# shadygm/Lichtfeld-Densification-Plugin

Measured on AMD Instinct MI355X. Metric: triangulated points/sec + pairs/sec, MipNeRF360 garden @fast, 1/2/4/8 GPU, higher is better.
Workload: dtype f32 (+f64 Sampson/DLT solve)

## Files before the change

### lichtfeld-densification-plugin_amd/csrc/lfd_api.hip

```cpp
#include <cstddef>
#include <hip/hip_runtime.h>
#include <hip/hip_ext.h>

#include <algorithm>
#include <cmath>
#include <cstdio>
#include <cstdlib>
#include <cstring>
#include <mutex>
#include <string>
#include <vector>

#include "lfd_context.hpp"
#include "lfd_corr.hpp"
#include "lfd_block.hpp"
#include "lfd_head.hpp"
#include "lfd_cycle.hpp"
#include "lfd_support.hpp"
#include "lfd_refine.hpp"
#include "lfd_normals.hpp"
#include "lfd_sigma.hpp"
#include "lfd_consensus.hpp"
#include "lfd_undistort.hpp"
#include "lfd_freespace.hpp"
#include "lfd_fuse.hpp"
#include "lfd_knn.hpp"
#include "lfd_cap.hpp"

extern "C" __global__ void lfd_aggregate_kernel(LfdLaunch L, float* best_cert, uint8_t* best_slot);
extern "C" __global__ void lfd_dense_kernel(LfdLaunch L);
extern "C" __global__ void lfd_dense_exact_kernel(LfdLaunch L);
extern "C" __global__ void lfd_dense_ply_kernel(LfdLaunch L);
extern "C" __global__ void lfd_dense_ply_exact_kernel(LfdLaunch L);
extern "C" __global__ void lfd_dense_segments_kernel(LfdLaunch L);
extern "C" __global__ void lfd_dense_segments_exact_kernel(LfdLaunch L);
extern "C" __global__ void lfd_dense_ply_segments_kernel(LfdLaunch L);
extern "C" __global__ void lfd_dense_ply_segments_exact_kernel(LfdLaunch L);
extern "C" __global__ void lfd_segment_scan_kernel(const LfdTileSeg* table, int n_tiles, int tiles_per_ref, int n_refs, long long* tile_dst, long long* ref_offsets);
extern "C" __global__ void lfd_order_segments_kernel(const long long* tile_dst, const LfdTileSeg* table, long long hw, int tiles_per_ref, int n_tiles,
                                                     const float* sxyz, const float* srgb, const float* serr, const int* scell, const unsigned char* sslot,
                                                     float* dxyz, float* drgb, float* derr, int* dcell, unsigned char* dslot, long long capacity);
extern "C" __global__ void lfd_pack_ply_segments_kernel(const long long* tile_dst, const LfdTileSeg* table, long long hw, int tiles_per_ref, int n_tiles,
                                                        const float* xyz, const float* rgb, long long capacity, unsigned char* out);
extern "C" __global__ void lfd_pack_points3d_segments_kernel(const long long* tile_dst, const LfdTileSeg* table, long long hw, int tiles_per_ref, int n_tiles,
                                                             const float* xyz, const float* rgb, const float* err, long long capacity,
                                                             unsigned long long id_base, unsigned char* out);
extern "C" __global__ void lfd_pair_setup_kernel(LfdLaunch L, LfdRefConst* ref_out, LfdPairConst* pair_out);
extern "C" __global__ void lfd_select_filter_kernel(LfdSelectArgs A);
extern "C" __global__ void lfd_pack_ply_kernel(const float* xyz, const float* rgb, long long n, unsigned char* out);
extern "C" __global__ void lfd_pack_points3d_kernel(const float* xyz, const float* rgb, const float* err, long long n,
                                                    unsigned long long id_base, unsigned char* out);
extern "C" __global__ void lfd_copy_segments_kernel(LfdCopyArgs A, const unsigned char* src, unsigned char* dst);
extern "C" __global__ void lfd_quantise_rgb_kernel(const float* rgb, long long n3, unsigned char* out);
extern "C" __global__ void lfd_voxel_minmax_kernel(const float* xyz, const float* rgb, long long n, LfdVoxStats* part);
extern "C" __global__ void lfd_voxel_final_kernel(const LfdVoxStats* part, int n_part, LfdVoxStats* out);
extern "C" __global__ void lfd_voxel_keys_kernel(const float* xyz, long long n, double o0, double o1, double o2, double vs, unsigned long long e1,
                                                 unsigned long long e2, unsigned long long* keys, unsigned* idx);
extern "C" __global__ void lfd_voxel_hist_kernel(const unsigned long long* keys, long long n, long long chunk, int shift, unsigned* counts);
extern "C" __global__ void lfd_voxel_scan_kernel(unsigned* v, int m, unsigned* total);
extern "C" __global__ void lfd_voxel_scatter_kernel(const unsigned long long* kin, const unsigned* iin, long long n, long long chunk, int shift,
                                                    const unsigned* counts, unsigned long long* kout, unsigned* iout);
extern "C" __global__ void lfd_voxel_head_count_kernel(const unsigned long long* keys, long long n, long long chunk, unsigned* counts);
extern "C" __global__ void lfd_voxel_head_scatter_kernel(const unsigned long long* keys, long long n, long long chunk, const unsigned* counts,
                                                         unsigned* vstart);
extern "C" __global__ void lfd_voxel_sums_kernel(const float* xyz, const float* rgb, long long n, const unsigned* sorted_idx, const unsigned* vstart,
                                                 const unsigned* nv_p, double cscale, float* xyz_out, float* rgb_out, unsigned* big, unsigned* n_big);
extern "C" __global__ void lfd_voxel_sums_big_kernel(const float* xyz, const float* rgb, long long n, const unsigned* sorted_idx, const unsigned* vstart,
                                                     const unsigned* nv_p, double cscale, const unsigned* big, const unsigned* n_big, float* xyz_out,
                                                     float* rgb_out);
hipError_t lfd_undistort_launch(const LfdUndistortArgs& p, unsigned long long* n_invalid, hipStream_t stream);
extern "C" __global__ void lfd_consensus_minmax_kernel(const float* xyz, long long n, LfdVoxStats* part);
extern "C" __global__ void lfd_consensus_keys_kernel(const float* xyz, long long n, double o0, double o1, double o2, double h, unsigned long long e1,
                                                     unsigned long long e2, unsigned long long sentinel, unsigned long long* keys, unsigned* idx);
extern "C" __global__ void lfd_consensus_gather_kernel(const float* xyz, const unsigned* sorted_idx, const long long* offs, int n_refs, long long n,
                                                       LfdConsensusPt* spt);
extern "C" __global__ void lfd_consensus_count_kernel(const unsigned long long* skey, const LfdConsensusPt* spt, const unsigned* sorted_idx, long long n,
                                                      unsigned long long e1, unsigned long long e2, unsigned long long sentinel, float r2, int min_refs,
                                                      int bound, uint8_t* keep, uint8_t* consensus);
extern "C" __global__ void lfd_consensus_wgcount_kernel(const uint8_t* keep, long long n, unsigned* wg_kept);
extern "C" __global__ void lfd_consensus_offsets_kernel(const long long* offs, int n_refs, const uint8_t* keep, const unsigned* wg_kept, long long* offs_out);
extern "C" __global__ void lfd_consensus_scatter_kernel(const float* xyz, const float* rgb, const float* err, long long n, const uint8_t* keep,
                                                        const unsigned* wg_kept, float* o_xyz, float* o_rgb, float* o_err);
extern "C" __global__ void lfd_fuse_side_kernel(const float* normals, long long n, const unsigned* sorted_idx, const unsigned* vstart, const unsigned* nv_p,
                                                uint8_t* flag, unsigned* rows, unsigned* big, unsigned* n_big);
extern "C" __global__ void lfd_fuse_side_big_kernel(const float* normals, long long n, const unsigned* sorted_idx, const unsigned* vstart, const unsigned* nv_p,
                                                    const unsigned* big, const unsigned* n_big, uint8_t* flag, unsigned* rows);
extern "C" __global__ void lfd_fuse_rowsum_kernel(const unsigned* rows, const unsigned* nv_p, long long chunk, unsigned* counts);
extern "C" __global__ void lfd_fuse_rowstart_kernel(unsigned* rows, const unsigned* nv_p, long long chunk, const unsigned* counts);
extern "C" __global__ void lfd_fuse_sums_kernel(const float* xyz, const float* normals, const float* rgb, long long n, const unsigned* sorted_idx,
                                                const unsigned* vstart, const unsigned* nv_p, const uint8_t* flag, const unsigned* rowstart, double cscale,
                                                float* xyz_out, float* normals_out, float* rgb_out, unsigned* count_out);
extern "C" __global__ void lfd_fuse_sums_big_kernel(const float* xyz, const float* normals, const float* rgb, long long n, const unsigned* sorted_idx,
                                                    const unsigned* vstart, const unsigned* nv_p, const uint8_t* flag, const unsigned* rowstart, double cscale,
                                                    const unsigned* big, const unsigned* n_big, float* xyz_out, float* normals_out, float* rgb_out,
                                                    unsigned* count_out);
extern "C" __global__ void lfd_knn_keys_kernel(const float* xyz, long long n, LfdKnnGrid g, unsigned long long* keys, unsigned* idx);
extern "C" __global__ void lfd_knn_cellmax_kernel(const unsigned* vstart, const unsigned* nv_p, long long n, unsigned* max_out);
extern "C" __global__ void lfd_knn_gather_kernel(const float* xyz, const unsigned* sorted_idx, long long n, LfdKnnPt* spt);
extern "C" __global__ void lfd_knn_scan_kernel(const unsigned long long* skey, const LfdKnnPt* spt, long long n, LfdKnnGrid g, float* dist2, unsigned* list,
                                               unsigned* n_list);
extern "C" __global__ void lfd_knn_brute_kernel(const LfdKnnPt* spt, long long n, const unsigned* list, const unsigned* n_list, float* dist2);
extern "C" __global__ void lfd_pack_gaussians_kernel(const float* xyz, const float* normals, const float* rgb, const float* dist2, long long n, float opacity,
                                                     double log_flatten, float max_m, float* out);
extern "C" __global__ void lfd_cap_keys_kernel(const float* xyz, long long n, LfdCapBox box, unsigned long long* keys, unsigned* idx);
extern "C" __global__ void lfd_cap_levels_kernel(const unsigned long long* keys, long long n, unsigned* hist);
extern "C" __global__ void lfd_cap_coarsen_kernel(unsigned long long* keys, long long n, int shift);
extern "C" __global__ void lfd_cap_rep_kernel(const unsigned* sorted_idx, const unsigned* vstart, const unsigned* nc_p, const float* err, long long n,
                                              unsigned long long budget, unsigned long long* rep);
extern "C" __global__ void lfd_cap_mark_kernel(const unsigned long long* rep, const unsigned* nc_p, long long n, unsigned long long budget, uint8_t* keep);
extern "C" __global__ void lfd_cap_index_kernel(const uint8_t* keep, const unsigned* wg_kept, long long n, long long capacity, long long* keep_out);
extern "C" __global__ void lfd_freespace_fill_kernel(uint32_t* zbuf, long long n_words);
extern "C" __global__ void lfd_freespace_splat_kernel(const float* xyz, long long n, const long long* offs, int n_refs, const LfdFreespaceCam* cams, int pw,
                                                      int ph, uint32_t* zbuf);
extern "C" __global__ void lfd_freespace_count_kernel(const float* xyz, long long n, const long long* offs, int n_refs, const LfdFreespaceCam* cams,
                                                      const uint32_t* zbuf, int pw, int ph, float tol, int min_violations, uint8_t* keep,
                                                      uint8_t* violations, uint8_t* supports);
hipError_t lfd_corr_launch(const LfdCorrArgs& p, hipStream_t stream);
hipError_t lfd_block_launch(const LfdBlockArgs& p, hipStream_t stream);
hipError_t lfd_head_launch(const LfdHeadArgs& p, hipStream_t stream);
hipError_t lfd_cycle_launch(const LfdCycleArgs& p, hipStream_t stream);
hipError_t lfd_support_launch(const LfdSupportArgs& p, hipStream_t stream);
hipError_t lfd_refine_launch(const LfdRefineArgs& p, hipStream_t stream);
hipError_t lfd_sigma_launch(const LfdSigmaArgs& p, hipStream_t stream);
hipError_t lfd_normals_launch(const LfdNormalArgs& p, hipStream_t stream);
extern "C" __global__ void lfd_pack_ply_normals_kernel(const float* xyz, const float* normals, const float* rgb, long long n, unsigned char* out);
extern "C" __global__ void lfd_select_topm_kernel(LfdSelectArgs A);
extern "C" __global__ void lfd_select_filter_mw_kernel(LfdSelectArgs A, LfdSelectNorms norms);
extern "C" __global__ void lfd_select_begins_kernel(long long* pairs, long long stride, int n);
extern "C" __global__ void lfd_mt_seed_kernel(unsigned* mt, unsigned seed);
extern "C" __global__ void lfd_mt_seed_batch_kernel(unsigned* mt_base, LfdSeedBatch seeds);
extern "C" __global__ void lfd_indexed_eval_kernel(LfdLaunch L, const long long* sel_idx, const long long* sel_offsets, float* scratch,
                                                   uint8_t* codes, unsigned* tab, int off_pairs);
extern "C" __global__ void lfd_indexed_kernel(LfdLaunch L, const long long* sel_idx, const long long* sel_offsets,
                                              float* scratch, uint8_t* codes, int32_t* seg_order, const unsigned* tab, int off_pairs);

namespace {

std::mutex g_create_mutex;
std::string g_create_error;
thread_local std::string t_create_error_copy;

}

namespace {

int fail(lfd_context* ctx, int code, const std::string& msg) { return lfd_fail(ctx, code, msg); }

#define LFD_HIP(ctx, expr)                                                                         \
    do {                                                                                           \
        hipError_t e_ = (expr);                                                                    \
        if (e_ != hipSuccess)                                                                      \
            return fail((ctx), LFD_ERR_HIP, std::string(#expr) + ": " + hipGetErrorString(e_));    \
    } while (0)

int ensure(lfd_context* ctx, DeviceBuffer& b, size_t bytes, bool zero = false) {
    if (b.bytes >= bytes && b.ptr) return LFD_OK;
    if (b.ptr) {
        LFD_HIP(ctx, hipStreamSynchronize(ctx->stream));
        if (ctx->prep_stream) LFD_HIP(ctx, hipStreamSynchronize(ctx->prep_stream));
        LFD_HIP(ctx, hipFree(b.ptr));
        b.ptr = nullptr; b.bytes = 0;
    }
    size_t want = std::max<size_t>(bytes, 256);
    want = (want + 255) & ~size_t(255);
    LFD_HIP(ctx, hipMalloc(&b.ptr, want));
    b.bytes = want;
    if (zero) LFD_HIP(ctx, hipMemsetAsync(b.ptr, 0, want, ctx->stream));
    return LFD_OK;
}

int validate_batch(lfd_context* ctx, const lfd_batch* b, const lfd_params* p) {
    if (!ctx) return fail(nullptr, LFD_ERR_INVALID, "null context");
    if (ctx->is_host) return fail(ctx, LFD_ERR_STATE, "this context was made by lfd_create_host: it serves the *_host entry points only");
    if (!b || !p) return fail(ctx, LFD_ERR_INVALID, "null batch/params");
    if (ctx->n_cams <= 0) return fail(ctx, LFD_ERR_STATE, "lfd_upload_cameras must be called first");
    if (b->n_refs <= 0) return fail(ctx, LFD_ERR_INVALID, "n_refs must be > 0");
    if (b->k <= 0 || b->k > LFD_MAX_SLOTS) return fail(ctx, LFD_ERR_INVALID, "k must be in [1, LFD_MAX_SLOTS]");
    if (b->H <= 0 || b->W <= 0 || b->w_match <= 1 || b->h_match <= 1) return fail(ctx, LFD_ERR_INVALID, "bad grid / match size");
    if (b->w_match >= (1 << 24) || b->h_match >= (1 << 24) || (long long)b->w_match * b->h_match * 3 > 0x7fffffffLL)
        return fail(ctx, LFD_ERR_INVALID, "match-size image too large");
    if ((long long)b->H * b->W > 0x7fffffffLL) return fail(ctx, LFD_ERR_INVALID, "grid too large");
    if (b->warp_channels != 2 && b->warp_channels != 4) return fail(ctx, LFD_ERR_INVALID, "warp_channels must be 2 or 4");
    if (!b->ref_cam || !b->n_slots || !b->nbr_cam || !b->cert || !b->warp || !b->image)
        return fail(ctx, LFD_ERR_INVALID, "null table in batch");
    if ((b->axis_x == nullptr) != (b->axis_y == nullptr)) return fail(ctx, LFD_ERR_INVALID, "axis_x and axis_y must both be given or both be null");
    for (int r = 0; r < b->n_refs; ++r) {
        if (b->ref_cam[r] < 0 || b->ref_cam[r] >= ctx->n_cams) return fail(ctx, LFD_ERR_INVALID, "ref_cam out of range");
        if (b->n_slots[r] < 1 || b->n_slots[r] > b->k) return fail(ctx, LFD_ERR_INVALID, "n_slots must be in [1, k]");
        if (!b->image[r]) return fail(ctx, LFD_ERR_INVALID, "null image pointer");
        for (int j = 0; j < b->n_slots[r]; ++j) {
            const size_t s = (size_t)r * b->k + j;
            if (b->nbr_cam[s] < 0 || b->nbr_cam[s] >= ctx->n_cams) return fail(ctx, LFD_ERR_INVALID, "nbr_cam out of range");
            if (!b->cert[s] || !b->warp[s]) return fail(ctx, LFD_ERR_INVALID, "null cert/warp pointer in a valid slot");
            if ((reinterpret_cast<uintptr_t>(b->cert[s]) & 15u) || (reinterpret_cast<uintptr_t>(b->warp[s]) & 15u))
                return fail(ctx, LFD_ERR_INVALID, "cert/warp planes must be 16-byte aligned");
        }
    }
    return LFD_OK;
}

int slot_events(lfd_context* ctx, LfdBatchSlot& sl) {
    if (!sl.pinned_free) LFD_HIP(ctx, hipEventCreateWithFlags(&sl.pinned_free, hipEventDisableTiming));
    if (!sl.ready) LFD_HIP(ctx, hipEventCreateWithFlags(&sl.ready, hipEventDisableTiming));
    if (!sl.idle) LFD_HIP(ctx, hipEventCreateWithFlags(&sl.idle, hipEventDisableTiming));
    return LFD_OK;
}

int upload_tables(lfd_context* ctx, const lfd_batch* b, const long long* extra, size_t n_extra, bool ahead, int* slot_out, hipStream_t* stream_out,
                  const LfdRefDesc** d_refs, const LfdSlotDesc** d_slots, const long long** d_extra, const float** d_fund) {
    const size_t nr = (size_t)b->n_refs, ns = nr * (size_t)b->k;
    const size_t off_slots = (nr * sizeof(LfdRefDesc) + 15) & ~size_t(15);
    const size_t off_fund = (off_slots + ns * sizeof(LfdSlotDesc) + 15) & ~size_t(15);
    const size_t total = (off_fund + (b->fundamental ? ns * 9 * sizeof(float) : 0) + 15) & ~size_t(15);
    const size_t off_extra = total;
    const size_t extra_room = ((nr + 1) * sizeof(long long) + 15) & ~size_t(15);
    std::vector<unsigned char> blob(total, 0);
    LfdRefDesc* refs = reinterpret_cast<LfdRefDesc*>(blob.data());
    LfdSlotDesc* slots = reinterpret_cast<LfdSlotDesc*>(blob.data() + off_slots);
    for (size_t r = 0; r < nr; ++r) {
        refs[r].image = b->image[r];
        refs[r].mask_a = b->mask_a ? b->mask_a[r] : nullptr;
        refs[r].cam = b->ref_cam[r];
        refs[r].n_slots = b->n_slots[r];
        refs[r].any_mask = refs[r].mask_a ? 1 : 0;
        refs[r].pad = 0;
        for (int j = 0; j < b->k; ++j) {
            LfdSlotDesc& s = slots[r * b->k + j];
            const bool valid = j < b->n_slots[r];
            s.cert = valid ? b->cert[r * b->k + j] : nullptr;
            s.warp = valid ? b->warp[r * b->k + j] : nullptr;
            s.mask_b = (valid && b->mask_b) ? b->mask_b[r * b->k + j] : nullptr;
            s.cam = valid ? b->nbr_cam[r * b->k + j] : 0;
            s.pad = 0;
            if (s.mask_b) refs[r].any_mask = 1;
        }
    }
    if (b->fundamental) std::memcpy(blob.data() + off_fund, b->fundamental, ns * 9 * sizeof(float));
    if (n_extra * sizeof(long long) > extra_room) return fail(ctx, LFD_ERR_INVALID, "internal: selection offsets beyond the reserved room");

    int si = -1;
    for (int c = 0; c < 2; ++c) {
        const int i = c == 0 ? ctx->cur : 1 - ctx->cur;
        if (ctx->slot[i].desc.ptr && ctx->slot[i].cache == blob) { si = i; break; }
    }
    hipStream_t st = ctx->stream;
    if (si >= 0) {
        LfdBatchSlot& sl = ctx->slot[si];
        if (!ahead && sl.ready_pending) {
#if !defined(LFD_EXPERIMENT_NO_READY_WAIT)
            LFD_HIP(ctx, hipStreamWaitEvent(ctx->stream, sl.ready, 0));
#endif
            sl.ready_pending = false;
        }
        if (ahead && sl.ready_pending) st = ctx->prep_stream;
    } else {
        if (ahead) {
            if (!ctx->prep_stream) LFD_HIP(ctx, hipStreamCreateWithFlags(&ctx->prep_stream, hipStreamNonBlocking));
            si = ctx->last_used < 0 ? ctx->cur : 1 - ctx->cur;
            st = ctx->prep_stream;
        } else {
            si = ctx->cur;
        }
        LfdBatchSlot& sl = ctx->slot[si];
        int rc = slot_events(ctx, sl);
        if (rc != LFD_OK) return rc;
        if (ahead) {
            if (sl.used) LFD_HIP(ctx, hipStreamWaitEvent(st, sl.idle_attached ? sl.idle_ext : sl.idle, 0));
        } else if (sl.ready_pending) {
            LFD_HIP(ctx, hipStreamWaitEvent(ctx->stream, sl.ready, 0));
            sl.ready_pending = false;
        }
        rc = ensure(ctx, sl.desc, total + extra_room);
        if (rc != LFD_OK) return rc;
        if (sl.pinned_bytes < total + extra_room) {
            if (sl.pinned_in_flight) { LFD_HIP(ctx, hipEventSynchronize(sl.pinned_free)); sl.pinned_in_flight = false; }
            if (sl.pinned) LFD_HIP(ctx, hipHostFree(sl.pinned));
            sl.pinned = nullptr;
            sl.pinned_bytes = std::max<size_t>((total + extra_room) * 2, 1 << 16);
            LFD_HIP(ctx, hipHostMalloc(&sl.pinned, sl.pinned_bytes, hipHostMallocDefault));
        }
        if (sl.pinned_in_flight) { LFD_HIP(ctx, hipEventSynchronize(sl.pinned_free)); sl.pinned_in_flight = false; }
        std::memcpy(sl.pinned, blob.data(), total);
        LFD_HIP(ctx, hipMemcpyAsync(sl.desc.ptr, sl.pinned, total, hipMemcpyHostToDevice, st));
        LFD_HIP(ctx, hipEventRecord(sl.pinned_free, st));
        sl.pinned_in_flight = true;
        sl.cache.swap(blob);
        sl.consts_valid = false;
    }
    LfdBatchSlot& sl = ctx->slot[si];
    if (n_extra) {
        if (sl.desc.bytes < total + extra_room) return fail(ctx, LFD_ERR_STATE, "internal: batch slot without room for the selection offsets");
        if (sl.x_in_flight) { LFD_HIP(ctx, hipEventSynchronize(sl.x_free)); sl.x_in_flight = false; }
        if (sl.pinned_x_bytes < extra_room) {
            if (sl.pinned_x) LFD_HIP(ctx, hipHostFree(sl.pinned_x));
            sl.pinned_x = nullptr;
            sl.pinned_x_bytes = std::max<size_t>(extra_room * 2, 4096);
            LFD_HIP(ctx, hipHostMalloc(&sl.pinned_x, sl.pinned_x_bytes, hipHostMallocDefault));
        }
        if (!sl.x_free) LFD_HIP(ctx, hipEventCreateWithFlags(&sl.x_free, hipEventDisableTiming));
        std::memcpy(sl.pinned_x, extra, n_extra * sizeof(long long));
        LFD_HIP(ctx, hipMemcpyAsync(static_cast<unsigned char*>(sl.desc.ptr) + off_extra, sl.pinned_x, n_extra * sizeof(long long), hipMemcpyHostToDevice,
                                    ctx->stream));
        LFD_HIP(ctx, hipEventRecord(sl.x_free, ctx->stream));
        sl.x_in_flight = true;
    }
    *slot_out = si;
    *stream_out = st;
    *d_refs = reinterpret_cast<const LfdRefDesc*>(sl.desc.ptr);
    *d_slots = reinterpret_cast<const LfdSlotDesc*>(static_cast<unsigned char*>(sl.desc.ptr) + off_slots);
    if (d_extra) *d_extra = reinterpret_cast<const long long*>(static_cast<unsigned char*>(sl.desc.ptr) + off_extra);
    *d_fund = b->fundamental ? reinterpret_cast<const float*>(static_cast<unsigned char*>(sl.desc.ptr) + off_fund) : nullptr;
    return LFD_OK;
}

int default_axes(lfd_context* ctx, int W, int H, const float** ax, const float** ay) {
    if (ctx->axes_w != W || ctx->axes_h != H || !ctx->axes.ptr) {
        int rc = ensure(ctx, ctx->axes, sizeof(float) * (size_t)(W + H));
        if (rc != LFD_OK) return rc;
        std::vector<float> host((size_t)W + H);
        lfd_identity_axis(W, host.data());
        lfd_identity_axis(H, host.data() + W);
        LFD_HIP(ctx, hipMemcpyAsync(ctx->axes.ptr, host.data(), host.size() * sizeof(float), hipMemcpyHostToDevice, ctx->stream));
        LFD_HIP(ctx, hipStreamSynchronize(ctx->stream));
        ctx->axes_w = W; ctx->axes_h = H;
    }
    *ax = static_cast<const float*>(ctx->axes.ptr);
    *ay = *ax + W;
    return LFD_OK;
}

int colour_tables(lfd_context* ctx, int W, int H, int wm, int hm, const LfdColourCol** cols, const LfdColourRow** rows) {
    const int key[4] = {W, H, wm, hm};
    if (!ctx->colour_tab.ptr || std::memcmp(key, ctx->colour_key, sizeof(key)) != 0) {
        static_assert(sizeof(LfdColourCol) == 16 && sizeof(LfdColourRow) == 16, "colour table entries are 16 bytes");
        int rc = ensure(ctx, ctx->colour_tab, sizeof(LfdColourCol) * (size_t)W + sizeof(LfdColourRow) * (size_t)H);
        if (rc != LFD_OK) return rc;
        std::vector<unsigned char> host(sizeof(LfdColourCol) * (size_t)W + sizeof(LfdColourRow) * (size_t)H);
        LfdColourCol* hc = reinterpret_cast<LfdColourCol*>(host.data());
        LfdColourRow* hr = reinterpret_cast<LfdColourRow*>(host.data() + sizeof(LfdColourCol) * (size_t)W);
        const LfdAxis ax = lfd_make_axis(W), ay = lfd_make_axis(H);
        for (int x = 0; x < W; ++x) hc[x] = lfd_colour_col(lfd_match_px(lfd_axis_value(ax, x), (float)(wm - 1)), wm);
        for (int y = 0; y < H; ++y) hr[y] = lfd_colour_row(lfd_match_px(lfd_axis_value(ay, y), (float)(hm - 1)), wm, hm);
        LFD_HIP(ctx, hipMemcpyAsync(ctx->colour_tab.ptr, host.data(), host.size(), hipMemcpyHostToDevice, ctx->stream));
        LFD_HIP(ctx, hipStreamSynchronize(ctx->stream));
        std::memcpy(ctx->colour_key, key, sizeof(key));
    }
    *cols = static_cast<const LfdColourCol*>(ctx->colour_tab.ptr);
    *rows = reinterpret_cast<const LfdColourRow*>(static_cast<const unsigned char*>(ctx->colour_tab.ptr) + sizeof(LfdColourCol) * (size_t)W);
    return LFD_OK;
}

}

void lfd_fill_kernel_params(const lfd_batch* b, const lfd_params* p, LfdKernelParams& kp) {
    kp.sampson_thresh = p->sampson_thresh;
    kp.certainty_thresh = p->certainty_thresh;
    kp.reproj_thresh = p->reproj_thresh;
    kp.no_filter = p->no_filter ? 1 : 0;
    (void)LFD_FLAG_EXACT_COLOUR;
    kp.use_sampson = (!p->no_filter && p->sampson_thresh > 0.0) ? 1 : 0;
    kp.use_parallax = (!p->no_filter && p->min_parallax_deg > 0.0f) ? 1 : 0;
    kp.dot_thresh = kp.use_parallax ? lfd_parallax_dot_threshold(p->min_parallax_deg) : 2.0f;
    kp.wm1 = (float)(b->w_match - 1);
    kp.hm1 = (float)(b->h_match - 1);
}

namespace {

int prepare_launch(lfd_context* ctx, const lfd_batch* b, const lfd_params* p, const long long* extra, size_t n_extra,
                   LfdLaunch& L, const long long** d_extra, bool ahead = false) {
    int rc = validate_batch(ctx, b, p);
    if (rc != LFD_OK) return rc;
    LFD_HIP(ctx, hipSetDevice(ctx->device));
    std::memset(&L, 0, sizeof(L));
    if (!ahead && ctx->last_used >= 0) {
        LfdBatchSlot& prev = ctx->slot[ctx->last_used];
        rc = slot_events(ctx, prev);
        if (rc != LFD_OK) return rc;
        if (!prev.idle_attached) LFD_HIP(ctx, hipEventRecord(prev.idle, ctx->stream));
        prev.used = true;
    }
    int si = 0;
    hipStream_t st = ctx->stream;
    rc = upload_tables(ctx, b, extra, n_extra, ahead, &si, &st, &L.refs, &L.slots, d_extra, &L.fund_override);
    if (rc != LFD_OK) return rc;
    LfdBatchSlot& sl = ctx->slot[si];
    L.cams = static_cast<const LfdCam*>(ctx->cams.ptr);
    if (b->axis_x) { L.axis_x = b->axis_x; L.axis_y = b->axis_y; }
    else {
        rc = default_axes(ctx, b->W, b->H, &L.axis_x, &L.axis_y);
        if (rc != LFD_OK) return rc;
        L.axis_identity = 1;
    }
    L.ax = lfd_make_axis(b->W);
    L.ay = lfd_make_axis(b->H);
    L.n_refs = b->n_refs; L.k = b->k; L.H = b->H; L.W = b->W;
    L.w_match = b->w_match; L.h_match = b->h_match; L.warp_channels = b->warp_channels;
    const long long HW = (long long)b->H * b->W;
    const int tile = LFD_DENSE_BLOCK * LFD_DENSE_CPT;
    L.tiles_per_ref = (int)((HW + tile - 1) / tile);
    L.mask_sx = (float)b->w_match / (float)b->W;
    L.mask_sy = (float)b->h_match / (float)b->H;
    L.inv_w = 1.0f / (float)b->W;
    L.w_log2 = -1;
    if ((b->W & (b->W - 1)) == 0) { int l = 0; while ((1 << l) < b->W) ++l; L.w_log2 = l; }
    lfd_fill_kernel_params(b, p, L.kp);
    const size_t ref_bytes = ((size_t)b->n_refs * sizeof(LfdRefConst) + 15) & ~size_t(15);
    const size_t need = ref_bytes + (size_t)b->n_refs * b->k * sizeof(LfdPairConst);
    if (sl.consts.bytes < need) sl.consts_valid = false;
    rc = ensure(ctx, sl.consts, need);
    if (rc != LFD_OK) return rc;
    LfdRefConst* d_rc = static_cast<LfdRefConst*>(sl.consts.ptr);
    LfdPairConst* d_pc = reinterpret_cast<LfdPairConst*>(static_cast<unsigned char*>(sl.consts.ptr) + ref_bytes);
    L.ref_const = d_rc;
    L.pair_const = d_pc;
    if (!sl.consts_valid || sl.wm != b->w_match || sl.hm != b->h_match) {
        const int n = b->n_refs * b->k + b->n_refs;
        hipLaunchKernelGGL(lfd_pair_setup_kernel, dim3((unsigned)((n + 63) / 64)), dim3(64), 0, st, L, d_rc, d_pc);
        LFD_HIP(ctx, hipGetLastError());
        sl.consts_valid = true;
        sl.refs = b->n_refs; sl.k = b->k;
        sl.wm = b->w_match;
        sl.hm = b->h_match;
        if (st != ctx->stream) {
            LFD_HIP(ctx, hipEventRecord(sl.ready, st));
            sl.ready_pending = true;
        }
    }
    if (!ahead) {
        ctx->cur = si; ctx->last_used = si;
        sl.idle_attached = false;
    }
    return LFD_OK;
}

constexpr size_t kWsHeader = 128 + 128 * LFD_TICKET_LANES;

int prepare_lookback(lfd_context* ctx, size_t n_tiles, size_t n_tickets, bool lanes, LfdLaunch& L) {
    const size_t need = kWsHeader + n_tiles * sizeof(unsigned long long);
    const bool fresh = ctx->ws.bytes < need || !ctx->ws.ptr;
    int rc = ensure(ctx, ctx->ws, need, true);
    if (rc != LFD_OK) return rc;
    if (fresh) {
        ctx->tickets_issued = 0; ctx->epoch = 0;
        for (int s = 0; s < LFD_TICKET_LANES; ++s) ctx->lane_issued[s] = 0;
    }
    ctx->epoch = (ctx->epoch + 1) & LFD_EPOCH_MASK;
    if (ctx->epoch == 0) {
        LFD_HIP(ctx, hipMemsetAsync(static_cast<unsigned char*>(ctx->ws.ptr) + kWsHeader, 0, ctx->ws.bytes - kWsHeader, ctx->stream));
        LFD_HIP(ctx, hipMemsetAsync(static_cast<unsigned char*>(ctx->ws.ptr) + 16, 0, 4, ctx->stream));
        ctx->epoch = 1;
    }
    unsigned char* base = static_cast<unsigned char*>(ctx->ws.ptr);
    L.ticket = reinterpret_cast<unsigned long long*>(base);
    L.ticket_lanes = reinterpret_cast<unsigned long long*>(base + 128);
    L.tile_state = reinterpret_cast<unsigned long long*>(base + kWsHeader);
    L.status = reinterpret_cast<unsigned int*>(base + 8);
    L.seg_ready = reinterpret_cast<unsigned int*>(base + 16);
    L.ticket_base = ctx->tickets_issued;
    L.epoch = ctx->epoch;
    if (lanes) {
        for (int s = 0; s < LFD_TICKET_LANES; ++s) {
            L.ticket_base_lane[s] = ctx->lane_issued[s];
            if ((size_t)s < n_tickets) ctx->lane_issued[s] += (n_tickets - (size_t)s + LFD_TICKET_LANES - 1) / LFD_TICKET_LANES;
        }
    } else {
        ctx->tickets_issued += n_tickets;
    }
    return LFD_OK;
}

void read_env_switches(lfd_context* ctx) {
    ctx->env = LfdEnvSwitches();
    if (const char* e = std::getenv("LFD_DENSE_EXTRA_LDS")) ctx->env.dense_extra_lds = (size_t)std::atol(e);
    if (const char* e = std::getenv("LFD_DENSE_TIMING")) ctx->env.dense_timing_path = e;
    if (const char* e = std::getenv("LFD_INDEXED_SPLIT")) ctx->env.indexed_split = std::atoi(e) != 0;
    if (const char* e = std::getenv("LFD_SELECT_TIMING")) ctx->env.select_timing = std::max(1, std::atoi(e));
    if (const char* e = std::getenv("LFD_SELECT_WORKGROUPS")) ctx->env.select_workgroups = std::atoi(e);
}

int check_points(lfd_context* ctx, const lfd_points* out, const long long* ref_offsets) {
    if (!out || !out->xyz || !out->rgb || !out->err) return fail(ctx, LFD_ERR_INVALID, "null output buffers");
    if (out->capacity < 0) return fail(ctx, LFD_ERR_INVALID, "negative capacity");
    if (!ref_offsets) return fail(ctx, LFD_ERR_INVALID, "ref_offsets is required");
    return LFD_OK;
}

int batch_launch(lfd_context* ctx, const lfd_batch* batch, LfdLaunch& L) {
    lfd_params none;
    std::memset(&none, 0, sizeof(none));
    return prepare_launch(ctx, batch, &none, nullptr, 0, L, nullptr);
}

struct CloudPlan {
    long long n;
    long long G, chunk;
    int n_part;
    long long n_wg;
    unsigned grid;
};

CloudPlan cloud_plan(int64_t n) {
    CloudPlan p;
    p.n = n;
    p.G = std::min<long long>(1024, (n + 4095) / 4096);
    p.chunk = (((n + p.G - 1) / p.G) + 511) / 512 * 512;
    p.G = (n + p.chunk - 1) / p.chunk;
    p.n_part = (int)std::min<long long>(1024, (n + 255) / 256);
    p.n_wg = (n + 255) / 256;
    p.grid = (unsigned)std::min<long long>(p.n_wg, 4096);
    return p;
}

struct Bump {
    unsigned char* base;
    size_t at = 0;
    template <class T>
    T* take(size_t count, size_t extra_bytes = 0) {
        const size_t o = at;
        at = (at + count * sizeof(T) + extra_bytes + 255) & ~size_t(255);
        return base ? reinterpret_cast<T*>(base + o) : nullptr;
    }
};

template <class Layout>
int carve_cloud_ws(lfd_context* ctx, Layout&& layout) {
    Bump size{nullptr};
    layout(size);
    if (int rc = ensure(ctx, ctx->cloud_ws, size.at)) return rc;
    Bump b{static_cast<unsigned char*>(ctx->cloud_ws.ptr)};
    layout(b);
    return LFD_OK;
}

struct CloudSort {
    LfdVoxStats *part, *stats;
    unsigned* counters;
    unsigned* counts;
    unsigned long long* keys[2];
    unsigned* idx[2];
    unsigned* vstart;
};

CloudSort carve_sort(Bump& b, long long n, int n_counters, bool heads) {
    CloudSort w;
    w.part = b.take<LfdVoxStats>(1024);
    w.stats = b.take<LfdVoxStats>(1, (size_t)n_counters * sizeof(unsigned));
    w.counters = w.stats ? reinterpret_cast<unsigned*>(w.stats + 1) : nullptr;
    w.counts = b.take<unsigned>(256 * 1024);
    for (int i = 0; i < 2; ++i) w.keys[i] = b.take<unsigned long long>((size_t)n);
    for (int i = 0; i < 2; ++i) w.idx[i] = b.take<unsigned>((size_t)n);
    w.vstart = heads ? b.take<unsigned>((size_t)n) : nullptr;
    return w;
}

int cloud_stats(lfd_context* ctx, const CloudPlan& p, const CloudSort& w, const float* xyz, const float* rgb, LfdVoxStats& s) {
    hipStream_t st = ctx->stream;
    if (rgb) hipLaunchKernelGGL(lfd_voxel_minmax_kernel, dim3(p.n_part), dim3(256), 0, st, xyz, rgb, p.n, w.part);
    else hipLaunchKernelGGL(lfd_consensus_minmax_kernel, dim3(p.n_part), dim3(256), 0, st, xyz, p.n, w.part);
    hipLaunchKernelGGL(lfd_voxel_final_kernel, dim3(1), dim3(256), 0, st, w.part, p.n_part, w.stats);
    LFD_HIP(ctx, hipGetLastError());
    LFD_HIP(ctx, hipMemcpyAsync(ctx->pinned_words, w.stats, sizeof(LfdVoxStats), hipMemcpyDeviceToHost, st));
    LFD_HIP(ctx, hipStreamSynchronize(st));
    std::memcpy(&s, ctx->pinned_words, sizeof(s));
    return LFD_OK;
}

int cloud_sort(hipStream_t st, const CloudPlan& p, const CloudSort& w, int bits) {
    int cur = 0;
    for (int shift = 0; shift < bits; shift += 8, cur ^= 1) {
        hipLaunchKernelGGL(lfd_voxel_hist_kernel, dim3((unsigned)p.G), dim3(256), 0, st, w.keys[cur], p.n, p.chunk, shift, w.counts);
        hipLaunchKernelGGL(lfd_voxel_scan_kernel, dim3(1), dim3(1024), 0, st, w.counts, (int)(256 * p.G), (unsigned*)nullptr);
        hipLaunchKernelGGL(lfd_voxel_scatter_kernel, dim3((unsigned)p.G), dim3(512), 0, st, w.keys[cur], w.idx[cur], p.n, p.chunk, shift, w.counts,
                           w.keys[cur ^ 1], w.idx[cur ^ 1]);
    }
    return cur;
}

void cloud_heads_count(hipStream_t st, const CloudPlan& p, const CloudSort& w, int cur) {
// ... 339 lines not shown
        if (FILE* f = std::fopen(stamp_path, "wb")) { std::fwrite(host.data(), sizeof(unsigned long long), host.size(), f); std::fclose(f); }
    }
#endif
    return LFD_OK;
}

int lfd_triangulate_dense(lfd_context* ctx, const lfd_batch* batch, const lfd_params* params, const lfd_points* out,
                          int64_t* ref_offsets, int32_t* seg_counts) {
    return dense_launch(ctx, batch, params, out, ref_offsets, seg_counts, nullptr, nullptr);
}

int lfd_triangulate_dense_ply(lfd_context* ctx, const lfd_batch* batch, const lfd_params* params, uint8_t* records, int64_t capacity,
                              int64_t* ref_offsets, int32_t* seg_counts, int32_t* cell, uint8_t* slot) {
    if (ctx && !records) return fail(ctx, LFD_ERR_INVALID, "lfd_triangulate_dense_ply: records is null");
    lfd_points out;
    std::memset(&out, 0, sizeof(out));
    out.capacity = capacity;
    out.cell = cell;
    out.slot = slot;
    return dense_launch(ctx, batch, params, &out, ref_offsets, seg_counts, nullptr, nullptr, records);
}

int lfd_dense_tiles_per_ref(int32_t H, int32_t W) {
    if (H <= 0 || W <= 0) return 0;
    const long long tile = LFD_DENSE_BLOCK * LFD_DENSE_CPT;
    return (int)(((long long)H * W + tile - 1) / tile);
}

int lfd_triangulate_dense_segments(lfd_context* ctx, const lfd_batch* batch, const lfd_params* params, const lfd_points* out,
                                   int64_t* ref_counts, int32_t* seg_counts, lfd_tile_segment* table) {
    if (ctx && !table) return fail(ctx, LFD_ERR_INVALID, "lfd_triangulate_dense_segments: the tile table is required");
    return dense_launch(ctx, batch, params, out, nullptr, seg_counts, ref_counts, table);
}

int lfd_triangulate_dense_ply_segments(lfd_context* ctx, const lfd_batch* batch, const lfd_params* params, uint8_t* records, int64_t capacity,
                                       int64_t* ref_counts, int32_t* seg_counts, lfd_tile_segment* table) {
    if (ctx && (!records || !table)) return fail(ctx, LFD_ERR_INVALID, "lfd_triangulate_dense_ply_segments: records and the tile table are required");
    lfd_points out;
    std::memset(&out, 0, sizeof(out));
    out.capacity = capacity;
    return dense_launch(ctx, batch, params, &out, nullptr, seg_counts, ref_counts, table, records);
}

static int segment_scan(lfd_context* ctx, int32_t n_refs, int32_t H, int32_t W, const lfd_tile_segment* table, int64_t* ref_offsets,
                        const long long** tile_dst, int* tpr_out, int* n_tiles_out) {
    if (!ctx) return fail(nullptr, LFD_ERR_INVALID, "null context");
    if (ctx->is_host) return fail(ctx, LFD_ERR_STATE, "device entry point called on a host context");
    if (n_refs <= 0 || H <= 0 || W <= 0 || !table) return fail(ctx, LFD_ERR_INVALID, "bad segment arguments");
    const int tpr = lfd_dense_tiles_per_ref(H, W);
    const long long n_tiles = (long long)n_refs * tpr;
    if (n_tiles > 0x7fffffffLL) return fail(ctx, LFD_ERR_INVALID, "too many tiles");
    LFD_HIP(ctx, hipSetDevice(ctx->device));
    int rc = ensure(ctx, ctx->seg_scan, ((size_t)n_tiles + 1) * sizeof(long long) + ((size_t)n_tiles + 2) * sizeof(int));
    if (rc != LFD_OK) return rc;
    long long* dst = static_cast<long long*>(ctx->seg_scan.ptr);
    hipLaunchKernelGGL(lfd_segment_scan_kernel, dim3(1), dim3(1024), 0, ctx->stream, reinterpret_cast<const LfdTileSeg*>(table), (int)n_tiles, tpr,
                       (int)n_refs, dst, reinterpret_cast<long long*>(ref_offsets));
    LFD_HIP(ctx, hipGetLastError());
    *tile_dst = dst; *tpr_out = tpr; *n_tiles_out = (int)n_tiles;
    return LFD_OK;
}

int lfd_order_segments(lfd_context* ctx, int32_t n_refs, int32_t H, int32_t W, const lfd_tile_segment* table, const lfd_points* src,
                       const lfd_points* dst, int64_t* ref_offsets) {
    const long long* tile_dst = nullptr; int tpr = 0, n_tiles = 0;
    int rc = segment_scan(ctx, n_refs, H, W, table, ref_offsets, &tile_dst, &tpr, &n_tiles);
    if (rc != LFD_OK) return rc;
    if (!src || !dst || !src->xyz || !src->rgb || !src->err || !dst->xyz || !dst->rgb || !dst->err) return fail(ctx, LFD_ERR_INVALID, "null point buffers");
    if (dst->capacity <= 0) return LFD_OK;
    const unsigned grid = (unsigned)std::min<int64_t>((dst->capacity + 1023) / 1024, 8192);
    hipLaunchKernelGGL(lfd_order_segments_kernel, dim3(grid), dim3(256), 0, ctx->stream, tile_dst, reinterpret_cast<const LfdTileSeg*>(table),
                       (long long)H * W, tpr, n_tiles, src->xyz, src->rgb, src->err, src->cell, src->slot, dst->xyz, dst->rgb, dst->err, dst->cell,
                       dst->slot, (long long)dst->capacity);
    LFD_HIP(ctx, hipGetLastError());
    return LFD_OK;
}

int lfd_pack_ply_segments(lfd_context* ctx, int32_t n_refs, int32_t H, int32_t W, const lfd_tile_segment* table, const float* xyz,
                          const float* rgb, int64_t capacity, uint8_t* out, int64_t* ref_offsets) {
    const long long* tile_dst = nullptr; int tpr = 0, n_tiles = 0;
    int rc = segment_scan(ctx, n_refs, H, W, table, ref_offsets, &tile_dst, &tpr, &n_tiles);
    if (rc != LFD_OK) return rc;
    if (capacity < 0 || (capacity > 0 && (!xyz || !rgb || !out))) return fail(ctx, LFD_ERR_INVALID, "bad arguments");
    if (reinterpret_cast<uintptr_t>(out) & 3u) return fail(ctx, LFD_ERR_INVALID, "out must be 4-byte aligned");
    if (capacity == 0) return LFD_OK;
    const unsigned grid = (unsigned)std::min<int64_t>((capacity + 255) / 256, 4096);
    hipLaunchKernelGGL(lfd_pack_ply_segments_kernel, dim3(grid), dim3(256), 0, ctx->stream, tile_dst, reinterpret_cast<const LfdTileSeg*>(table),
                       (long long)H * W, tpr, n_tiles, xyz, rgb, (long long)capacity, out);
    LFD_HIP(ctx, hipGetLastError());
    return LFD_OK;
}

int lfd_pack_points3d_segments(lfd_context* ctx, int32_t n_refs, int32_t H, int32_t W, const lfd_tile_segment* table, const float* xyz,
                               const float* rgb, const float* err, int64_t capacity, uint64_t id_base, uint8_t* out, int64_t* ref_offsets) {
    const long long* tile_dst = nullptr; int tpr = 0, n_tiles = 0;
    int rc = segment_scan(ctx, n_refs, H, W, table, ref_offsets, &tile_dst, &tpr, &n_tiles);
    if (rc != LFD_OK) return rc;
    if (capacity < 0 || (capacity > 0 && (!xyz || !rgb || !err || !out))) return fail(ctx, LFD_ERR_INVALID, "bad arguments");
    if (reinterpret_cast<uintptr_t>(out) & 3u) return fail(ctx, LFD_ERR_INVALID, "out must be 4-byte aligned");
    if (capacity == 0) return LFD_OK;
    const unsigned grid = (unsigned)std::min<int64_t>((capacity + 255) / 256, 4096);
    hipLaunchKernelGGL(lfd_pack_points3d_segments_kernel, dim3(grid), dim3(256), 0, ctx->stream, tile_dst, reinterpret_cast<const LfdTileSeg*>(table),
                       (long long)H * W, tpr, n_tiles, xyz, rgb, err, (long long)capacity, (unsigned long long)id_base, out);
    LFD_HIP(ctx, hipGetLastError());
    return LFD_OK;
}

int lfd_triangulate_indexed(lfd_context* ctx, const lfd_batch* batch, const lfd_params* params, const int64_t* sel_idx,
                            const int64_t* sel_offsets, const lfd_points* out, int64_t* ref_offsets, int32_t* seg_counts,
                            int32_t* seg_order) {
    if (ctx && (!sel_idx || !sel_offsets)) return fail(ctx, LFD_ERR_INVALID, "sel_idx / sel_offsets are required");
    if (ctx && batch && batch->n_refs > 0) {
        if (sel_offsets[0] != 0) return fail(ctx, LFD_ERR_INVALID, "sel_offsets[0] must be 0");
        for (int r = 0; r < batch->n_refs; ++r)
            if (sel_offsets[r + 1] < sel_offsets[r]) return fail(ctx, LFD_ERR_INVALID, "sel_offsets must be non-decreasing");
    }
    LfdLaunch L;
    const long long* d_off = nullptr;
    int rc = prepare_launch(ctx, batch, params, reinterpret_cast<const long long*>(sel_offsets),
                            batch ? (size_t)std::max(batch->n_refs, 0) + 1 : 0, L, &d_off);
    if (rc != LFD_OK) return rc;
    rc = check_points(ctx, out, reinterpret_cast<long long*>(ref_offsets));
    if (rc != LFD_OK) return rc;
    const size_t n_sel = (size_t)sel_offsets[batch->n_refs];
    rc = prepare_lookback(ctx, (size_t)batch->n_refs, (size_t)batch->n_refs, false, L);
    if (rc != LFD_OK) return rc;
    rc = ensure(ctx, ctx->scratch, std::max<size_t>(n_sel, 1) * 8 * sizeof(float));
    if (rc != LFD_OK) return rc;
    rc = ensure(ctx, ctx->codes, std::max<size_t>(n_sel, 1));
    if (rc != LFD_OK) return rc;
    L.xyz = out->xyz; L.rgb = out->rgb; L.err = out->err; L.cell = out->cell; L.slot = out->slot;
    L.capacity = out->capacity;
    L.ref_offsets = reinterpret_cast<long long*>(ref_offsets);
    L.seg_counts = seg_counts;
    bool split = true;
    split = ctx->env.indexed_split;
    long long max_sel = 0;
    for (int r = 0; r < batch->n_refs; ++r) max_sel = std::max<long long>(max_sel, sel_offsets[r + 1] - sel_offsets[r]);
    unsigned* tab = nullptr;
    if (split && max_sel > 0) {
        const size_t tab_bytes = (size_t)batch->n_refs * LFD_MAX_SLOTS * 2 * sizeof(unsigned);
        rc = ensure(ctx, ctx->idx_tab, tab_bytes);
        if (rc != LFD_OK) return rc;
        tab = static_cast<unsigned*>(ctx->idx_tab.ptr);
        LFD_HIP(ctx, hipMemsetAsync(tab, 0, tab_bytes, ctx->stream));
        const unsigned chunks = (unsigned)((max_sel + LFD_INDEXED_EVAL_BLOCK - 1) / LFD_INDEXED_EVAL_BLOCK);
        hipLaunchKernelGGL(lfd_indexed_eval_kernel, dim3(chunks, (unsigned)batch->n_refs), dim3(LFD_INDEXED_EVAL_BLOCK), 0, ctx->stream, L,
                           reinterpret_cast<const long long*>(sel_idx), d_off, static_cast<float*>(ctx->scratch.ptr),
                           static_cast<uint8_t*>(ctx->codes.ptr), tab, 0);
        LFD_HIP(ctx, hipGetLastError());
    }
    hipLaunchKernelGGL(lfd_indexed_kernel, dim3((unsigned)batch->n_refs), dim3(LFD_INDEXED_BLOCK), 0, ctx->stream, L,
                       reinterpret_cast<const long long*>(sel_idx), d_off, static_cast<float*>(ctx->scratch.ptr),
                       static_cast<uint8_t*>(ctx->codes.ptr), seg_order, static_cast<const unsigned*>(tab), 0);
    LFD_HIP(ctx, hipGetLastError());
    return LFD_OK;
}

int lfd_rng_seed(lfd_context* ctx, uint32_t seed) {
    if (!ctx) return fail(nullptr, LFD_ERR_INVALID, "null context");
    if (ctx->is_host) return fail(ctx, LFD_ERR_STATE, "device entry point called on a host context");
    LFD_HIP(ctx, hipSetDevice(ctx->device));
    int rc = ensure(ctx, ctx->mt, 625 * sizeof(unsigned));
    if (rc != LFD_OK) return rc;
    hipLaunchKernelGGL(lfd_mt_seed_kernel, dim3(1), dim3(64), 0, ctx->stream, static_cast<unsigned*>(ctx->mt.ptr), seed);
    LFD_HIP(ctx, hipGetLastError());
    ctx->mt_seeded = true;
    return LFD_OK;
}

int lfd_rng_get_state(lfd_context* ctx, uint32_t* key624, int32_t* pos) {
    if (!ctx || !key624 || !pos) return fail(ctx, LFD_ERR_INVALID, "null argument");
    if (ctx->is_host) return fail(ctx, LFD_ERR_STATE, "device entry point called on a host context");
    if (!ctx->mt_seeded) return fail(ctx, LFD_ERR_STATE, "lfd_rng_seed / lfd_rng_set_state must be called first");
    unsigned host[625];
    LFD_HIP(ctx, hipSetDevice(ctx->device));
    LFD_HIP(ctx, hipMemcpyAsync(host, ctx->mt.ptr, sizeof(host), hipMemcpyDeviceToHost, ctx->stream));
    LFD_HIP(ctx, hipStreamSynchronize(ctx->stream));
    std::memcpy(key624, host, 624 * sizeof(unsigned));
    *pos = (int32_t)host[624];
    return LFD_OK;
}

int lfd_rng_set_state(lfd_context* ctx, const uint32_t* key624, int32_t pos) {
    if (!ctx || !key624 || pos < 0 || pos > 624) return fail(ctx, LFD_ERR_INVALID, "bad MT19937 state");
    if (ctx->is_host) return fail(ctx, LFD_ERR_STATE, "device entry point called on a host context");
    LFD_HIP(ctx, hipSetDevice(ctx->device));
    int rc = ensure(ctx, ctx->mt, 625 * sizeof(unsigned));
    if (rc != LFD_OK) return rc;
    unsigned host[625];
    std::memcpy(host, key624, 624 * sizeof(unsigned));
    host[624] = (unsigned)pos;
    LFD_HIP(ctx, hipMemcpyAsync(ctx->mt.ptr, host, sizeof(host), hipMemcpyHostToDevice, ctx->stream));
    LFD_HIP(ctx, hipStreamSynchronize(ctx->stream));
    ctx->mt_seeded = true;
    return LFD_OK;
}

static int rng_checkpoint_copy(lfd_context* ctx, int32_t place, bool take_back) {
    if (!ctx) return fail(nullptr, LFD_ERR_INVALID, "null context");
    if (ctx->is_host) return fail(ctx, LFD_ERR_STATE, "device entry point called on a host context");
    if (place < 0 || place >= LFD_RNG_CHECKPOINTS) return fail(ctx, LFD_ERR_INVALID, "checkpoint place out of range");
    if (!ctx->mt_seeded) return fail(ctx, LFD_ERR_STATE, "lfd_rng_seed / lfd_rng_set_state must be called first");
    if (take_back && !(ctx->mt_ckpt_taken & (1u << place))) return fail(ctx, LFD_ERR_STATE, "no checkpoint was taken at this place");
    LFD_HIP(ctx, hipSetDevice(ctx->device));
    int rc = ensure(ctx, ctx->mt_ckpt, (size_t)LFD_RNG_CHECKPOINTS * 640 * sizeof(unsigned));
    if (rc != LFD_OK) return rc;
    unsigned* slot = static_cast<unsigned*>(ctx->mt_ckpt.ptr) + (size_t)place * 640;
    if (take_back) LFD_HIP(ctx, hipMemcpyAsync(ctx->mt.ptr, slot, 625 * sizeof(unsigned), hipMemcpyDeviceToDevice, ctx->stream));
    else LFD_HIP(ctx, hipMemcpyAsync(slot, ctx->mt.ptr, 625 * sizeof(unsigned), hipMemcpyDeviceToDevice, ctx->stream));
    if (!take_back) ctx->mt_ckpt_taken |= 1u << place;
    return LFD_OK;
}

int lfd_rng_checkpoint(lfd_context* ctx, int32_t place) { return rng_checkpoint_copy(ctx, place, false); }
int lfd_rng_rollback(lfd_context* ctx, int32_t place) { return rng_checkpoint_copy(ctx, place, true); }

static bool select_runs_on_several_workgroups(lfd_context* ctx, long long N) {
    int n_wg = LFD_SELECT_DEFAULT_WG;
    if (ctx->env.select_workgroups >= 0) n_wg = ctx->env.select_workgroups;
    n_wg = std::min(std::min(n_wg, (int)LFD_SELECT_MAX_WG), (int)(N / 8192));
    return n_wg >= 2 && ctx->env.select_timing == 0;
}

static int select_launch(lfd_context* ctx, bool topm, const float* best_cert, int32_t H, int32_t W, int32_t M, float cap,
                         int32_t border, int32_t tiles, float s_override, int64_t* sel_out, int64_t capacity,
                         long long* sel_offsets_dev, int** d_info, unsigned char** d_time, int n_batch = 1,
                         unsigned* mt_batch = nullptr, int* info_batch = nullptr, const float* s_batch = nullptr) {
    if (!ctx) return fail(nullptr, LFD_ERR_INVALID, "null context");
    if (!best_cert || !sel_out) return fail(ctx, LFD_ERR_INVALID, "null argument");
    if (ctx->is_host) return fail(ctx, LFD_ERR_STATE, "device entry point called on a host context");
    if (H <= 0 || W <= 0 || (long long)H * W > 0x7fffffffLL || M < 0 || tiles <= 0 || border < 0 || capacity < 0)
        return fail(ctx, LFD_ERR_INVALID, "bad selection arguments");
    if (!topm && !mt_batch && !ctx->mt_seeded) return fail(ctx, LFD_ERR_STATE, "lfd_rng_seed must be called before lfd_select_samples");
    if (n_batch < 1 || n_batch > LFD_SELECT_BATCH_MAX) return fail(ctx, LFD_ERR_INVALID, "bad selection batch");
    LFD_HIP(ctx, hipSetDevice(ctx->device));
    if (!ctx->mt.ptr) { int rc0 = ensure(ctx, ctx->mt, 625 * sizeof(unsigned)); if (rc0 != LFD_OK) return rc0; }
    const size_t N = (size_t)H * W, Mz = (size_t)std::max(M, 1);
    auto up = [](size_t v) { return (v + 255) & ~size_t(255); };
    const size_t o_w = 0, o_p = o_w + up(N * 4), o_cdf = o_p + up(N * 8), o_first = o_cdf + up(N * 8), o_mark = o_first + up(N * 4),
                 o_draws = o_mark + up(N), o_cand = o_draws + up(Mz * 8), o_found = o_cand + up(Mz * 4), o_out = o_found + up(Mz * 4),
                 o_time = o_out + 256, o_coop = o_time + 256, total = o_coop + up(LFD_SELECT_COOP_BYTES);
    int rc = ensure(ctx, ctx->sel_scratch, total * (size_t)n_batch);
    if (rc != LFD_OK) return rc;
    unsigned char* base = static_cast<unsigned char*>(ctx->sel_scratch.ptr);
    LfdSelectArgs A;
    std::memset(&A, 0, sizeof(A));
    A.best_cert = best_cert;
    A.weights = reinterpret_cast<float*>(base + o_w);
    A.p = reinterpret_cast<double*>(base + o_p);
    A.cdf = reinterpret_cast<double*>(base + o_cdf);
    A.first = reinterpret_cast<int*>(base + o_first);
    A.mark = base + o_mark;
    A.draws = reinterpret_cast<double*>(base + o_draws);
    A.cand = reinterpret_cast<int*>(base + o_cand);
    A.found = reinterpret_cast<int*>(base + o_found);
    A.mt = mt_batch ? mt_batch : static_cast<unsigned*>(ctx->mt.ptr);
    A.batch_scratch_stride = (long long)total;
    A.batch_cert_stride = (long long)N;
    A.batch_out_stride = (long long)capacity;
    A.batch_mt_stride = mt_batch ? LFD_MT_STATE_STRIDE : 0;
    A.batch_info = info_batch;
    A.sel_out = reinterpret_cast<long long*>(sel_out);
    A.n_out = reinterpret_cast<int*>(base + o_out);
    A.status = reinterpret_cast<int*>(base + o_out + 4);
    A.capacity = capacity;
    A.H = H; A.W = W; A.M = M; A.border = border; A.tiles = tiles; A.cap = cap; A.s_override = s_override;
    A.sel_offsets_out = sel_offsets_dev;
    LfdSelectNorms norms;
    std::memset(&norms, 0, sizeof(norms));
    if (s_batch) {
        norms.use = 1;
        for (int i = 0; i < n_batch; ++i) norms.s[i] = s_batch[i];
    }
    *d_info = reinterpret_cast<int*>(base + o_out);
    *d_time = nullptr;
    const bool timing = !topm && n_batch == 1 && ctx->env.select_timing != 0;
    if (timing) {
        A.timing = reinterpret_cast<unsigned long long*>(base + o_time);
        LFD_HIP(ctx, hipMemsetAsync(base + o_time, 0, 256, ctx->stream));
        *d_time = base + o_time;
    }
    if (topm) {
        const size_t lds = (size_t)LFD_SELECT_TOPM_MAX * sizeof(unsigned long long);
        if (!ctx->topm_lds_attr_set) {
            LFD_HIP(ctx, hipFuncSetAttribute(reinterpret_cast<const void*>(lfd_select_topm_kernel),
                                             hipFuncAttributeMaxDynamicSharedMemorySize, (int)lds));
            ctx->topm_lds_attr_set = true;
        }
        hipLaunchKernelGGL(lfd_select_topm_kernel, dim3(1, (unsigned)n_batch), dim3(LFD_SELECT_BLOCK), lds, ctx->stream, A);
    } else {
        int n_wg = LFD_SELECT_DEFAULT_WG;
        if (ctx->env.select_workgroups >= 0) n_wg = ctx->env.select_workgroups;
        n_wg = std::min(std::min(n_wg, (int)LFD_SELECT_MAX_WG), (int)(N / 8192));
        {
            const int tile = std::max(1, W / tiles);
            const long long nbins = (long long)((W - 1) / tile + 1) * ((H - 1) / tile + 1);
            if (nbins > LFD_SELECT_MAX_BINS)
                return fail(ctx, LFD_ERR_INVALID, "selection: too many coverage bins: a " + std::to_string(H) + " x " + std::to_string(W) + " grid with " +
                            std::to_string(tiles) + " tiles per side has " + std::to_string(nbins) + " coverage tiles, the device stage holds " +
                            std::to_string((int)LFD_SELECT_MAX_BINS) + " (every square grid fits; RoMa's, 320 ... 1280 cells per side, have 576 ... 625); the host selection "
                            "stage (selection_backend=\"host\" in the Python mirror: upstream's own library calls) has no such limit");
        }
        const bool timing_mw = timing && ctx->env.select_timing == 2;
        const bool several_wg = n_wg >= 2 && (!timing || timing_mw);
        const bool one_stream = mt_batch == nullptr;
        if (one_stream && n_batch > 1 && !several_wg)
            return fail(ctx, LFD_ERR_STATE, "selection: several references on one stream need the multi-workgroup kernel");
        if (several_wg) {
            const long long first_round = std::max<long long>(std::min<long long>((long long)((double)M * 0.85), (long long)N), 1);
            long long ring_cap = 4096;
            while (ring_cap < 4 * first_round) ring_cap *= 2;
            const int snap_slots = (int)(2 * ring_cap / 624) + 8;
            const size_t o_ring = LFD_CHAIN_BYTES, o_snaps = o_ring + (size_t)ring_cap * 8,
                         chain_total = (o_snaps + (size_t)snap_slots * 624 * 4 + 255) & ~size_t(255);
            const int n_chains = one_stream ? 1 : n_batch;
            rc = ensure(ctx, ctx->sel_chain, chain_total * (size_t)n_chains);
            if (rc != LFD_OK) return rc;
            unsigned char* cb = static_cast<unsigned char*>(ctx->sel_chain.ptr);
            if (n_chains == 1) LFD_HIP(ctx, hipMemsetAsync(cb, 0, LFD_CHAIN_BYTES, ctx->stream));
            else LFD_HIP(ctx, hipMemset2DAsync(cb, chain_total, 0, LFD_CHAIN_BYTES, (size_t)n_chains, ctx->stream));
            A.chain = cb;
            A.ring = reinterpret_cast<double*>(cb + o_ring);
            A.snaps = reinterpret_cast<unsigned*>(cb + o_snaps);
            A.ring_cap = ring_cap;
            A.snap_slots = snap_slots;
            A.chain_refs = one_stream ? n_batch : 1;
            A.batch_chain_stride = one_stream ? 0 : (long long)chain_total;
        }
        if (several_wg) {
            A.coop = base + o_coop;
            A.n_wg = n_wg;
            if (n_batch == 1) LFD_HIP(ctx, hipMemsetAsync(base + o_coop, 0, LFD_COOP_MT, ctx->stream));
            else LFD_HIP(ctx, hipMemset2DAsync(base + o_coop, total, 0, LFD_COOP_MT, (size_t)n_batch, ctx->stream));
            hipLaunchKernelGGL(lfd_select_filter_mw_kernel, dim3((unsigned)n_wg + 1u, (unsigned)n_batch), dim3(LFD_SELECT_BLOCK), 0, ctx->stream, A, norms);
        } else {
            hipLaunchKernelGGL(lfd_select_filter_kernel, dim3(1, (unsigned)n_batch), dim3(LFD_SELECT_BLOCK), 0, ctx->stream, A);
        }
    }
    LFD_HIP(ctx, hipGetLastError());
    return LFD_OK;
}

static const char* select_status_name(int st) {
    static const char* names[] = {"ok", "probabilities contain NaN", "probabilities are not non-negative",
                                  "Fewer non-zero entries in p than size", "weight below 2^-29: exact parallel cumsum not guaranteed",
                                  "no progress", "too many coverage bins", "sel_out capacity too small"};
    return names[std::min(std::max(st, 0), 7)];
}

static int select_impl(lfd_context* ctx, bool topm, const float* best_cert, int32_t H, int32_t W, int32_t M, float cap,
                       int32_t border, int32_t tiles, float s_override, int64_t* sel_out, int64_t capacity,
                       int32_t* n_sel_host, int32_t* status_host) {
    if (ctx && (!n_sel_host || !status_host)) return fail(ctx, LFD_ERR_INVALID, "null argument");
    int* d_info = nullptr;
    unsigned char* d_time = nullptr;
    int rc = select_launch(ctx, topm, best_cert, H, W, M, cap, border, tiles, s_override, sel_out, capacity, nullptr, &d_info, &d_time);
    if (rc != LFD_OK) return rc;
    int* host = ctx->pinned_words + 4;
    LFD_HIP(ctx, hipMemcpyAsync(host, d_info, 2 * sizeof(int), hipMemcpyDeviceToHost, ctx->stream));
    LFD_HIP(ctx, hipStreamSynchronize(ctx->stream));
    *n_sel_host = host[0];
    *status_host = host[1];
    if (d_time) {
        unsigned long long t[32];
        LFD_HIP(ctx, hipMemcpy(t, d_time, sizeof(t), hipMemcpyDeviceToHost));
        fprintf(stderr, "[lfd] select phases (us):");
        for (int i = 1; i < 30 && t[i]; ++i) fprintf(stderr, " %.1f", (double)(t[i] - t[i - 1]) * 0.01);
        if (t[30]) fprintf(stderr, " | stream workgroup: start +%.1f, first draws ready +%.1f", (double)((long long)t[30] - (long long)t[0]) * 0.01, (double)((long long)t[31] - (long long)t[0]) * 0.01);
        fprintf(stderr, "\n");
    }
    if (host[1] != LFD_SELECT_OK)
        return fail(ctx, host[1] == LFD_SELECT_CAPACITY ? LFD_ERR_CAPACITY : LFD_ERR_INVALID,
                    std::string("selection: ") + select_status_name(host[1]));
    return LFD_OK;
}

static int sampled_impl(lfd_context* ctx, const lfd_batch* batch, const lfd_params* params, int32_t M, float cap, int32_t border, int32_t tiles,
                        float s_override, const uint32_t* seeds, const lfd_points* out, int64_t* ref_offsets, int32_t* seg_counts,
                        int32_t* seg_order, int32_t* sel_info, int64_t* sel_cells, bool chain = false, const float* s_chain = nullptr) {
    if (!ctx) return fail(nullptr, LFD_ERR_INVALID, "null context");
    if (ctx->is_host) return fail(ctx, LFD_ERR_STATE, "device entry point called on a host context");
    if (!batch || !params || !sel_info) return fail(ctx, LFD_ERR_INVALID, "null argument");
    const int R = batch->n_refs;
    if (R != 1 && !seeds && !chain) return fail(ctx, LFD_ERR_INVALID, "lfd_triangulate_sampled takes one reference view per call (several: lfd_triangulate_sampled_chain on the context's stream, lfd_triangulate_sampled_multi on per-reference streams)");
    if (R < 1) return fail(ctx, LFD_ERR_INVALID, "no reference view");
    if (M < 0 || tiles <= 0 || border < 0) return fail(ctx, LFD_ERR_INVALID, "bad selection arguments");
    const bool topm = params->no_filter != 0;
    if (topm && M > LFD_SELECT_TOPM_MAX) return fail(ctx, LFD_ERR_INVALID, "no_filter selection is limited to 16384 matches per reference");
    LfdLaunch L;
    int rc = prepare_launch(ctx, batch, params, nullptr, 0, L, nullptr);
    if (rc != LFD_OK) return rc;
    rc = check_points(ctx, out, reinterpret_cast<long long*>(ref_offsets));
    if (rc != LFD_OK) return rc;
    const long long HW = (long long)batch->H * batch->W;
    const long long cap_sel = topm ? std::max<long long>(std::min<long long>(M, HW), 1) : (long long)M + (long long)tiles * tiles + 64;
    if (out->capacity < cap_sel * R) return fail(ctx, LFD_ERR_CAPACITY, "output capacity below (M + tiles*tiles + 64) per reference");
    rc = ensure(ctx, ctx->agg, (size_t)HW * (size_t)R * sizeof(float));
    if (rc != LFD_OK) return rc;
    float* best = static_cast<float*>(ctx->agg.ptr);
    {
        const int per_block = 256 * 4;
        const int gx = (int)std::min<long long>((HW + per_block - 1) / per_block, 2048);
        hipLaunchKernelGGL(lfd_aggregate_kernel, dim3((unsigned)gx, (unsigned)R, 1u), dim3(256), 0, ctx->stream, L, best, static_cast<uint8_t*>(nullptr));
        LFD_HIP(ctx, hipGetLastError());
    }
    rc = ensure(ctx, ctx->sel_buf, (size_t)R * 16 + (size_t)cap_sel * (size_t)R * sizeof(long long));
    if (rc != LFD_OK) return rc;
    long long* sel_pairs = static_cast<long long*>(ctx->sel_buf.ptr);
    long long* cells = sel_cells ? reinterpret_cast<long long*>(sel_cells) : sel_pairs + 2 * (size_t)R;
    if (R == 1) {
        LFD_HIP(ctx, hipMemsetAsync(sel_pairs, 0, 16, ctx->stream));
    } else {
        hipLaunchKernelGGL(lfd_select_begins_kernel, dim3((unsigned)((R + 255) / 256)), dim3(256), 0, ctx->stream, sel_pairs, (long long)cap_sel, R);
        LFD_HIP(ctx, hipGetLastError());
    }
    if (!seeds && (topm || select_runs_on_several_workgroups(ctx, HW)) && R > 1) {
        if (!topm && !ctx->mt_seeded) return fail(ctx, LFD_ERR_STATE, "lfd_rng_seed must be called before lfd_triangulate_sampled_chain");
        for (int r0 = 0; r0 < R; r0 += LFD_SELECT_BATCH_MAX) {
            const int nb = std::min(R - r0, (int)LFD_SELECT_BATCH_MAX);
            int* d_info = nullptr;
            unsigned char* d_time = nullptr;
            rc = select_launch(ctx, topm, best + (size_t)r0 * HW, batch->H, batch->W, M, cap, topm ? 0 : border, topm ? 1 : tiles, 0.0f,
                               reinterpret_cast<int64_t*>(cells + (size_t)r0 * cap_sel), cap_sel, sel_pairs + 2 * (size_t)r0, &d_info, &d_time,
                               nb, nullptr, sel_info + 2 * (size_t)r0, (s_chain && !topm) ? s_chain + r0 : nullptr);
            if (rc != LFD_OK) return rc;
        }
    } else if (!seeds) {
        for (int r = 0; r < R; ++r) {
            int* d_info = nullptr;
            unsigned char* d_time = nullptr;
            const float s_r = topm ? 0.0f : (s_chain ? s_chain[r] : s_override);
            rc = select_launch(ctx, topm, best + (size_t)r * HW, batch->H, batch->W, M, cap, topm ? 0 : border, topm ? 1 : tiles, s_r,
                               reinterpret_cast<int64_t*>(cells + (size_t)r * cap_sel), cap_sel, sel_pairs + 2 * (size_t)r, &d_info, &d_time);
            if (rc != LFD_OK) return rc;
            LFD_HIP(ctx, hipMemcpyAsync(sel_info + 2 * (size_t)r, d_info, 2 * sizeof(int), hipMemcpyDeviceToDevice, ctx->stream));
        }
    } else {
        rc = ensure(ctx, ctx->mt_batch, (size_t)LFD_SELECT_BATCH_MAX * LFD_MT_STATE_STRIDE * sizeof(unsigned));
        if (rc != LFD_OK) return rc;
        unsigned* mtb = static_cast<unsigned*>(ctx->mt_batch.ptr);
        for (int r0 = 0; r0 < R; r0 += LFD_SELECT_BATCH_MAX) {
            const int nb = std::min(R - r0, (int)LFD_SELECT_BATCH_MAX);
            if (!topm) {
                LfdSeedBatch sb;
                std::memset(&sb, 0, sizeof(sb));
                for (int i = 0; i < nb; ++i) sb.seed[i] = seeds[r0 + i];
                hipLaunchKernelGGL(lfd_mt_seed_batch_kernel, dim3((unsigned)nb), dim3(64), 0, ctx->stream, mtb, sb);
                LFD_HIP(ctx, hipGetLastError());
            }
            int* d_info = nullptr;
            unsigned char* d_time = nullptr;
            rc = select_launch(ctx, topm, best + (size_t)r0 * HW, batch->H, batch->W, M, cap, topm ? 0 : border, topm ? 1 : tiles, 0.0f,
                               reinterpret_cast<int64_t*>(cells + (size_t)r0 * cap_sel), cap_sel, sel_pairs + 2 * (size_t)r0, &d_info, &d_time,
                               nb, mtb, sel_info + 2 * (size_t)r0);
            if (rc != LFD_OK) return rc;
        }
    }
    rc = prepare_lookback(ctx, (size_t)R, (size_t)R, false, L);
    if (rc != LFD_OK) return rc;
    rc = ensure(ctx, ctx->scratch, (size_t)cap_sel * (size_t)R * 8 * sizeof(float));
    if (rc != LFD_OK) return rc;
    rc = ensure(ctx, ctx->codes, (size_t)cap_sel * (size_t)R);
    if (rc != LFD_OK) return rc;
    const size_t tab_bytes = (size_t)R * LFD_MAX_SLOTS * 2 * sizeof(unsigned);
    rc = ensure(ctx, ctx->idx_tab, tab_bytes);
    if (rc != LFD_OK) return rc;
    unsigned* tab = static_cast<unsigned*>(ctx->idx_tab.ptr);
    LFD_HIP(ctx, hipMemsetAsync(tab, 0, tab_bytes, ctx->stream));
    L.xyz = out->xyz; L.rgb = out->rgb; L.err = out->err; L.cell = out->cell; L.slot = out->slot;
    L.capacity = out->capacity;
    L.ref_offsets = reinterpret_cast<long long*>(ref_offsets);
    L.seg_counts = seg_counts;
    const unsigned chunks = (unsigned)((cap_sel + LFD_INDEXED_EVAL_BLOCK - 1) / LFD_INDEXED_EVAL_BLOCK);
    hipLaunchKernelGGL(lfd_indexed_eval_kernel, dim3(chunks, (unsigned)R), dim3(LFD_INDEXED_EVAL_BLOCK), 0, ctx->stream, L,
                       static_cast<const long long*>(cells), static_cast<const long long*>(sel_pairs), static_cast<float*>(ctx->scratch.ptr),
                       static_cast<uint8_t*>(ctx->codes.ptr), tab, 1);
    LFD_HIP(ctx, hipGetLastError());
    hipLaunchKernelGGL(lfd_indexed_kernel, dim3((unsigned)R), dim3(LFD_INDEXED_BLOCK), 0, ctx->stream, L,
                       static_cast<const long long*>(cells), static_cast<const long long*>(sel_pairs), static_cast<float*>(ctx->scratch.ptr),
                       static_cast<uint8_t*>(ctx->codes.ptr), seg_order, static_cast<const unsigned*>(tab), 1);
    LFD_HIP(ctx, hipGetLastError());
    LFD_HIP(ctx, hipMemcpyAsync(sel_info + 2 * (size_t)R, static_cast<unsigned char*>(ctx->ws.ptr) + 8, sizeof(int), hipMemcpyDeviceToDevice, ctx->stream));
    return LFD_OK;
}

int lfd_triangulate_sampled(lfd_context* ctx, const lfd_batch* batch, const lfd_params* params, int32_t M, float cap,
                            int32_t border, int32_t tiles, float s_override, const lfd_points* out, int64_t* ref_offsets,
                            int32_t* seg_counts, int32_t* seg_order, int32_t* sel_info, int64_t* sel_cells) {
    if (ctx && batch && batch->n_refs != 1) return fail(ctx, LFD_ERR_INVALID, "lfd_triangulate_sampled takes one reference view per call");
    return sampled_impl(ctx, batch, params, M, cap, border, tiles, s_override, nullptr, out, ref_offsets, seg_counts, seg_order, sel_info, sel_cells);
}

int lfd_triangulate_sampled_chain(lfd_context* ctx, const lfd_batch* batch, const lfd_params* params, int32_t M, float cap,
                                  int32_t border, int32_t tiles, const float* s_overrides, const lfd_points* out, int64_t* ref_offsets,
                                  int32_t* seg_counts, int32_t* seg_order, int32_t* sel_info, int64_t* sel_cells) {
    return sampled_impl(ctx, batch, params, M, cap, border, tiles, 0.0f, nullptr, out, ref_offsets, seg_counts, seg_order, sel_info, sel_cells, true, s_overrides);
}

int lfd_triangulate_sampled_multi(lfd_context* ctx, const lfd_batch* batch, const lfd_params* params, int32_t M, float cap,
                                  int32_t border, int32_t tiles, const uint32_t* seeds, const lfd_points* out, int64_t* ref_offsets,
                                  int32_t* seg_counts, int32_t* seg_order, int32_t* sel_info, int64_t* sel_cells) {
    if (ctx && !seeds) return fail(ctx, LFD_ERR_INVALID, "seeds is required: every reference draws from its own MT19937 stream");
    return sampled_impl(ctx, batch, params, M, cap, border, tiles, 0.0f, seeds, out, ref_offsets, seg_counts, seg_order, sel_info, sel_cells);
}

int lfd_select_samples(lfd_context* ctx, const float* best_cert, int32_t H, int32_t W, int32_t M, float cap,
                       int32_t border, int32_t tiles, float s_override, int64_t* sel_out, int64_t capacity,
                       int32_t* n_sel_host, int32_t* status_host) {
    return select_impl(ctx, false, best_cert, H, W, M, cap, border, tiles, s_override, sel_out, capacity, n_sel_host, status_host);
}

int lfd_select_top_m(lfd_context* ctx, const float* best_cert, int32_t H, int32_t W, int32_t M, float cap,
                     int64_t* sel_out, int64_t capacity, int32_t* n_sel_host, int32_t* status_host) {
    return select_impl(ctx, true, best_cert, H, W, M, cap, 0, 1, 0.0f, sel_out, capacity, n_sel_host, status_host);
}

int lfd_pack_ply(lfd_context* ctx, const float* xyz, const float* rgb, int64_t n, uint8_t* out) {
    if (!ctx) return fail(nullptr, LFD_ERR_INVALID, "null context");
    if (ctx->is_host) return fail(ctx, LFD_ERR_STATE, "device entry point called on a host context");
    if (n < 0 || (n > 0 && (!xyz || !rgb || !out))) return fail(ctx, LFD_ERR_INVALID, "bad arguments");
    if (reinterpret_cast<uintptr_t>(out) & 3u) return fail(ctx, LFD_ERR_INVALID, "out must be 4-byte aligned");
    if (n == 0) return LFD_OK;
    LFD_HIP(ctx, hipSetDevice(ctx->device));
    const unsigned grid = (unsigned)std::min<int64_t>((n + 255) / 256, 4096);
    hipLaunchKernelGGL(lfd_pack_ply_kernel, dim3(grid), dim3(256), 0, ctx->stream, xyz, rgb, (long long)n, out);
    LFD_HIP(ctx, hipGetLastError());
    return LFD_OK;
}

int lfd_pack_ply_normals(lfd_context* ctx, const float* xyz, const float* normals, const float* rgb, int64_t n, uint8_t* out) {
    if (!ctx) return fail(nullptr, LFD_ERR_INVALID, "null context");
    if (ctx->is_host) return fail(ctx, LFD_ERR_STATE, "device entry point called on a host context");
    if (n < 0 || (n > 0 && (!xyz || !normals || !rgb || !out))) return fail(ctx, LFD_ERR_INVALID, "bad arguments");
    if (reinterpret_cast<uintptr_t>(out) & 3u) return fail(ctx, LFD_ERR_INVALID, "out must be 4-byte aligned");
    if (n == 0) return LFD_OK;
    LFD_HIP(ctx, hipSetDevice(ctx->device));
    const unsigned grid = (unsigned)std::min<int64_t>((n + 255) / 256, 4096);
    hipLaunchKernelGGL(lfd_pack_ply_normals_kernel, dim3(grid), dim3(256), 0, ctx->stream, xyz, normals, rgb, (long long)n, out);
    LFD_HIP(ctx, hipGetLastError());
    return LFD_OK;
}

int lfd_pack_points3d(lfd_context* ctx, const float* xyz, const float* rgb, const float* err, int64_t n, uint64_t id_base,
                      uint8_t* out) {
    if (!ctx) return fail(nullptr, LFD_ERR_INVALID, "null context");
    if (ctx->is_host) return fail(ctx, LFD_ERR_STATE, "device entry point called on a host context");
    if (n < 0 || (n > 0 && (!xyz || !rgb || !out))) return fail(ctx, LFD_ERR_INVALID, "bad arguments");
    if (reinterpret_cast<uintptr_t>(out) & 3u) return fail(ctx, LFD_ERR_INVALID, "out must be 4-byte aligned");
    if (n == 0) return LFD_OK;
    LFD_HIP(ctx, hipSetDevice(ctx->device));
    const unsigned grid = (unsigned)std::min<int64_t>((n + 255) / 256, 4096);
    hipLaunchKernelGGL(lfd_pack_points3d_kernel, dim3(grid), dim3(256), 0, ctx->stream, xyz, rgb, err, (long long)n,
                       (unsigned long long)id_base, out);
    LFD_HIP(ctx, hipGetLastError());
    return LFD_OK;
}

int lfd_voxel_downsample(lfd_context* ctx, const float* xyz, const float* rgb, int64_t n, double voxel_size, float* xyz_out, float* rgb_out,
                         int64_t* n_out_host) {
    if (!ctx) return fail(nullptr, LFD_ERR_INVALID, "null context");
    if (ctx->is_host) return fail(ctx, LFD_ERR_STATE, "device entry point called on a host context");
    if (!n_out_host || n < 0 || (n > 0 && (!xyz || !rgb || !xyz_out || !rgb_out))) return fail(ctx, LFD_ERR_INVALID, "lfd_voxel_downsample: bad arguments");
    if (!(voxel_size > 0.0) || !std::isfinite(voxel_size)) return fail(ctx, LFD_ERR_INVALID, "lfd_voxel_downsample: voxel_size must be finite and > 0");
    if (n > 0x7fffffffLL) return fail(ctx, LFD_ERR_INVALID, "lfd_voxel_downsample: at most 2^31 - 1 points");
    *n_out_host = 0;
    if (n == 0) return LFD_OK;
    LFD_HIP(ctx, hipSetDevice(ctx->device));
    hipStream_t st = ctx->stream;
    const CloudPlan p = cloud_plan(n);
    CloudSort w;
    unsigned* big = nullptr;
    if (int rc = carve_cloud_ws(ctx, [&](Bump& b) {
            w = carve_sort(b, p.n, 2, true);
            big = b.take<unsigned>((size_t)n / (LFD_VOX_BIG + 1) + 1);
        }))
        return rc;
    unsigned *nv_dev = w.counters, *n_big = w.counters + 1;

    LfdVoxStats s;
    if (int rc = cloud_stats(ctx, p, w, xyz, rgb, s)) return rc;
    if (s.flags & LFD_VOX_NONFINITE) return fail(ctx, LFD_ERR_INVALID, "lfd_voxel_downsample: " LFD_FUSE_NONFINITE);
    LfdFuseGrid g;
    if (!lfd_fuse_grid(s.lo, s.hi, voxel_size, g)) return fail(ctx, LFD_ERR_INVALID, "lfd_voxel_downsample: " LFD_FUSE_KEY_RANGE);
    const double cscale = lfd_fuse_cscale(s.cmax, (s.flags & LFD_VOX_NAN_RGB) != 0u);

    hipLaunchKernelGGL(lfd_voxel_keys_kernel, dim3(p.grid), dim3(256), 0, st, xyz, p.n, g.origin[0], g.origin[1], g.origin[2], voxel_size, g.e[1],
                       g.e[2], w.keys[0], w.idx[0]);
    const int cur = cloud_sort(st, p, w, g.bits);
    cloud_heads_count(st, p, w, cur);
    cloud_heads_scatter(st, p, w, cur);
    LFD_HIP(ctx, hipMemsetAsync(n_big, 0, sizeof(unsigned), st));
    hipLaunchKernelGGL(lfd_voxel_sums_kernel, dim3(p.grid), dim3(256), 0, st, xyz, rgb, p.n, w.idx[cur], w.vstart, nv_dev, cscale, xyz_out, rgb_out,
                       big, n_big);
    const unsigned big_grid = (unsigned)std::min<long long>(n / (LFD_VOX_BIG + 1) + 1, 8192);
    hipLaunchKernelGGL(lfd_voxel_sums_big_kernel, dim3(big_grid), dim3(64), 0, st, xyz, rgb, p.n, w.idx[cur], w.vstart, nv_dev, cscale, big, n_big,
                       xyz_out, rgb_out);
    LFD_HIP(ctx, hipGetLastError());
    LFD_HIP(ctx, hipMemcpyAsync(ctx->pinned_words, nv_dev, sizeof(unsigned), hipMemcpyDeviceToHost, st));
    LFD_HIP(ctx, hipStreamSynchronize(st));
    *n_out_host = (int64_t)(unsigned)ctx->pinned_words[0];
    return LFD_OK;
}

int lfd_consensus_filter(lfd_context* ctx, const float* xyz, const float* rgb, const float* err, int64_t n, const int64_t* ref_offsets_host,
                         int32_t n_refs, float radius, int32_t min_refs, float* xyz_out, float* rgb_out, float* err_out,
                         int64_t* ref_offsets_out_host, uint8_t* consensus, int64_t* n_out_host) {
    if (!ctx) return fail(nullptr, LFD_ERR_INVALID, "null context");
    if (ctx->is_host) return fail(ctx, LFD_ERR_STATE, "device entry point called on a host context");
    if (const char* why = lfd_consensus_check(xyz, rgb, err, n, ref_offsets_host, n_refs, radius, min_refs, xyz_out, rgb_out, err_out,
                                              ref_offsets_out_host, consensus, n_out_host))
        return fail(ctx, LFD_ERR_INVALID, std::string("lfd_consensus_filter: ") + why);
    for (int32_t r = 0; r <= n_refs; ++r) ref_offsets_out_host[r] = 0;
    *n_out_host = 0;
    if (n == 0) return LFD_OK;
    LFD_HIP(ctx, hipSetDevice(ctx->device));
    hipStream_t st = ctx->stream;
    const CloudPlan p = cloud_plan(n);
    CloudSort w;
    LfdConsensusPt* spt = nullptr;
    CloudCompact c;
    if (int rc = carve_cloud_ws(ctx, [&](Bump& b) {
            w = carve_sort(b, p.n, 0, false);
            spt = b.take<LfdConsensusPt>((size_t)n);
            c = carve_compact(b, p, n_refs);
        }))
        return rc;

    LFD_HIP(ctx, hipMemcpyAsync(c.offs, ref_offsets_host, ((size_t)n_refs + 1) * sizeof(long long), hipMemcpyHostToDevice, st));
    LfdVoxStats s;
    if (int rc = cloud_stats(ctx, p, w, xyz, nullptr, s)) return rc;
    if (!(s.lo[0] <= s.hi[0])) {
        if (consensus) LFD_HIP(ctx, hipMemsetAsync(consensus, 0, (size_t)n, st));
        LFD_HIP(ctx, hipStreamSynchronize(st));
        return LFD_OK;
    }
// ... 610 lines not shown
```

### lichtfeld-densification-plugin_amd/csrc/lfd_device.hpp

```cpp
#pragma once

#include <stdint.h>

#include "lfd_geometry.hpp"

#ifndef LFD_MAX_SLOTS
#define LFD_MAX_SLOTS 16
#endif

#ifndef LFD_DENSE_BLOCK
#define LFD_DENSE_BLOCK 256
#endif
#ifndef LFD_COPY_UNROLL
#define LFD_COPY_UNROLL 2
#endif
#ifndef LFD_TICKET_LANES
#define LFD_TICKET_LANES 8
#endif
#define LFD_DENSE_CPT 4
#ifndef LFD_DENSE_WAVES_PER_SIMD
#define LFD_DENSE_WAVES_PER_SIMD 8
#endif
#ifndef LFD_DENSE_ALL_WARPS
#define LFD_DENSE_ALL_WARPS 0
// ... 42 lines not shown
    const uint8_t* mask_a;
    int32_t cam;
    int32_t n_slots;
    int32_t any_mask;
    int32_t pad;
};

struct LfdSlotDesc {
    const float* cert;
    const float* warp;
    const uint8_t* mask_b;
    int32_t cam;
    int32_t pad;
};

#define LFD_COPY_MAX_SEGS 96
#define LFD_COPY_CHUNK 32768
struct LfdCopyArgs {
    long long src[LFD_COPY_MAX_SEGS], dst[LFD_COPY_MAX_SEGS], n[LFD_COPY_MAX_SEGS];
    int chunk0[LFD_COPY_MAX_SEGS + 1];
    int n_segs;
};

struct LfdVoxStats {
    float lo[3], hi[3];
    float cmax;
    unsigned flags;
};
#define LFD_VOX_NONFINITE 1u
#define LFD_VOX_NAN_RGB 2u
#define LFD_VOX_BIG 64
struct LfdTileSeg { int32_t offset, count; };

struct LfdLaunch {
    const LfdCam* cams;
    const LfdRefDesc* refs;
    const LfdSlotDesc* slots;
    const LfdRefConst* ref_const;
    const LfdPairConst* pair_const;
    const float* axis_x;
    const float* axis_y;
    const float* fund_override;
    int32_t n_refs, k, H, W, w_match, h_match, warp_channels, tiles_per_ref;
    float mask_sx, mask_sy;
    float inv_w;
    int32_t axis_identity;
    LfdAxis ax, ay;
    int32_t w_log2;
    int32_t pad1;
    LfdKernelParams kp;
    float* xyz;
    float* rgb;
    float* err;
    int32_t* cell;
    uint8_t* slot;
    long long capacity;
    long long* ref_offsets;
    int32_t* seg_counts;
    unsigned long long* tile_state;
    unsigned long long* ticket;
    unsigned long long* ticket_lanes;
    unsigned long long ticket_base;
    unsigned long long ticket_base_lane[LFD_TICKET_LANES];
    unsigned int epoch;
    unsigned int pad0;
    unsigned int* status;
    unsigned int* seg_ready;
    const LfdColourCol* colour_cols;
    const LfdColourRow* colour_rows;
    unsigned long long* phase_stamps;
    unsigned long long* ref_cursor;
    LfdTileSeg* tile_table;
    unsigned char* ply;
};

#define LFD_SELECT_BLOCK 1024
#define LFD_SELECT_MAX_BINS 2304
#define LFD_SELECT_TOPM_MAX 16384
#ifndef LFD_SELECT_DEFAULT_WG
#define LFD_SELECT_DEFAULT_WG 16
#endif
#define LFD_SELECT_MAX_WG 64
#define LFD_COOP_BAR 0
#define LFD_COOP_FLAGS 16
#define LFD_COOP_MSG 32
#define LFD_COOP_PART 64
#define LFD_COOP_SPAN (LFD_COOP_PART + 8 * LFD_SELECT_MAX_WG)
#define LFD_COOP_WGCNT (LFD_COOP_SPAN + 8 * 16 * LFD_SELECT_MAX_WG)
#define LFD_COOP_BINS ((LFD_COOP_WGCNT + 4 * (LFD_SELECT_MAX_WG + 1) + 7) & ~7)
#define LFD_COOP_MT (LFD_COOP_BINS + 8 * LFD_SELECT_MAX_BINS)
#define LFD_SELECT_COOP_BYTES (LFD_COOP_MT + 4 * 640)
#define LFD_SELECT_OK 0
#define LFD_SELECT_NAN 1
#define LFD_SELECT_NEGATIVE 2
#define LFD_SELECT_FEWER_NONZERO 3
#define LFD_SELECT_INEXACT 4
#define LFD_SELECT_NO_PROGRESS 5
#define LFD_SELECT_TOO_MANY_BINS 6
#define LFD_SELECT_CAPACITY 7

#define LFD_SELECT_BATCH_MAX 32
struct LfdSelectArgs {
    const float* best_cert;
    float* weights;
    double* p;
    double* cdf;
    int* first;
    unsigned char* mark;
    double* draws;
    int* cand;
    int* found;
    unsigned* mt;
    long long* sel_out;
    int* n_out;
    int* status;
    long long capacity;
    int H, W, M, border, tiles;
    float cap;
    float s_override;
    unsigned long long* timing;
    unsigned char* coop;
    int n_wg;
    long long* sel_offsets_out;
    long long batch_scratch_stride;
    long long batch_cert_stride;
    long long batch_out_stride;
    long long batch_mt_stride;
    int* batch_info;
    unsigned char* chain;
    double* ring;
    unsigned* snaps;
    long long ring_cap;
    int snap_slots;
    int chain_refs;
    long long batch_chain_stride;
};
struct LfdSelectNorms {
    int use;
    float s[LFD_SELECT_BATCH_MAX];
};
#define LFD_MT_STATE_STRIDE 640
#define LFD_CHAIN_PRODUCED 0
#define LFD_CHAIN_WANT 8
#define LFD_CHAIN_RELEASED 16
#define LFD_CHAIN_STATE 24
#define LFD_CHAIN_CURRENT 28
#define LFD_CHAIN_OFF 64
#define LFD_CHAIN_BROKEN (~0ull)
#define LFD_CHAIN_BEG 384
#define LFD_CHAIN_TENT 656
#define LFD_CHAIN_BYTES 1024
struct LfdSeedBatch { unsigned seed[LFD_SELECT_BATCH_MAX]; };

#if defined(__HIPCC__)
#include "lfd_support.hpp"

struct LfdPointSpan {
    long long total, i, last, ii;
    bool any, mine;
};

__device__ __forceinline__ LfdPointSpan lfd_point_span(const long long* offs, int n_refs, long long capacity) {
    LfdPointSpan w;
    w.total = lfd_support_clamp(offs[n_refs], capacity);
    const long long base = (long long)blockIdx.x * 256;
    w.any = base < w.total;
    w.i = base + (int)threadIdx.x;
    w.mine = w.i < w.total;
    w.last = (base + 256 < w.total ? base + 256 : w.total) - 1;
    w.ii = w.mine ? w.i : w.last;
    return w;
}

__device__ __forceinline__ void lfd_stage_slots(LfdSlot* sh, const void* slots, const LfdPairConst* pair_const, int rr, int k, int ns) {
    const int tid = (int)threadIdx.x;
    if (tid < ns) {
        const LfdSlotDesc& d = static_cast<const LfdSlotDesc*>(slots)[(size_t)rr * k + tid];
        lfd_slot_fill(sh[tid], d.cert, d.warp, d.mask_b, pair_const[(size_t)rr * k + tid]);
    }
}
#endif
```

### lichtfeld-densification-plugin_amd/csrc/lfd_kernels.hip

```cpp
#include <hip/hip_runtime.h>
#include <stdint.h>

#include "lfd_device.hpp"

namespace {

constexpr int kBlock = LFD_DENSE_BLOCK;
constexpr int kCpt = LFD_DENSE_CPT;
constexpr int kTile = kBlock * kCpt;

typedef unsigned long long u64;

constexpr u64 kStEmpty = 0ull, kStAggregate = 1ull, kStPrefix = 2ull;
constexpr u64 kValueMask = (1ull << LFD_VALUE_BITS) - 1ull;
__device__ __forceinline__ u64 pack_state(u64 st, unsigned epoch, u64 v) {
    return (st << 62) | ((u64)epoch << LFD_VALUE_BITS) | (v & kValueMask);
}
__device__ __forceinline__ u64 state_status(u64 s, unsigned epoch) {
    return (((s >> LFD_VALUE_BITS) & LFD_EPOCH_MASK) == epoch) ? (s >> 62) : kStEmpty;
}

__device__ __forceinline__ void state_store(u64* p, u64 v) {
    __hip_atomic_store(p, v, __ATOMIC_RELAXED, __HIP_MEMORY_SCOPE_AGENT);
}
// ... 143 lines not shown
    unsigned* dst = reinterpret_cast<unsigned*>(S.pc);
    const int nw = L.k * (int)(sizeof(LfdPairConst) / 4);
#pragma unroll
    for (int q = 0; q < kPw; ++q) { const int i = tid + q * (int)blockDim.x; if (i < nw) dst[i] = P.pw[q]; }
    const int nsw = L.k * (int)(sizeof(LfdSlotDesc) / 4);
    if (tid < nsw) reinterpret_cast<unsigned*>(S.slot)[tid] = P.sw;
    if (tid < (int)(sizeof(LfdRefConst) / 4)) reinterpret_cast<unsigned*>(&S.rc)[tid] = P.rw;
    if (tid >= 64 && tid < 64 + (int)(sizeof(LfdRefDesc) / 4)) reinterpret_cast<unsigned*>(&S.ref)[tid - 64] = P.rw;
}

__device__ __forceinline__ void block_prologue(const LfdLaunch& L, int r, BlockShared& S) {
    const int tid = (int)threadIdx.x;
    {
        const unsigned* src = reinterpret_cast<const unsigned*>(L.pair_const + (size_t)r * L.k);
        unsigned* dst = reinterpret_cast<unsigned*>(S.pc);
        const int nw = L.k * (int)(sizeof(LfdPairConst) / 4);
        for (int i = tid; i < nw; i += (int)blockDim.x) dst[i] = src[i];
        const unsigned* ssrc = reinterpret_cast<const unsigned*>(L.slots + (size_t)r * L.k);
        unsigned* sdst = reinterpret_cast<unsigned*>(S.slot);
        const int nsw = L.k * (int)(sizeof(LfdSlotDesc) / 4);
        for (int i = tid; i < nsw; i += (int)blockDim.x) sdst[i] = ssrc[i];
        const unsigned* rsrc = reinterpret_cast<const unsigned*>(L.ref_const + r);
        unsigned* rdst = reinterpret_cast<unsigned*>(&S.rc);
        if (tid < (int)(sizeof(LfdRefConst) / 4)) rdst[tid] = rsrc[tid];
        const unsigned* dsrc = reinterpret_cast<const unsigned*>(L.refs + r);
        unsigned* ddst = reinterpret_cast<unsigned*>(&S.ref);
        if (tid >= 64 && tid < 64 + (int)(sizeof(LfdRefDesc) / 4)) ddst[tid - 64] = dsrc[tid - 64];
    }
    __syncthreads();
}

__device__ __forceinline__ void lfd_divmod(int cell, int W, float inv_w, int& y, int& x) {
    int q = (int)((float)cell * inv_w);
    int r = cell - q * W;
    if (r < 0) { --q; r += W; }
    if (r >= W) { ++q; r -= W; }
    if (r < 0) { --q; r += W; }
    if (r >= W) { ++q; r -= W; }
    y = q; x = r;
}

__device__ __forceinline__ void lfd_divmod_local(int local, int W, float inv_w, int w_log2, int& dy, int& x) {
    if (w_log2 >= 0) { dy = local >> w_log2; x = local & (W - 1); return; }
    int q = (int)((float)local * inv_w);
    int r = local - __mul24(q, W);
    if (r < 0) { --q; r += W; }
    if (r >= W) { ++q; r -= W; }
    dy = q; x = r;
}

__device__ __forceinline__ float cell_cert(const LfdLaunch& L, const BlockShared& S, int j, int cell, int x, int y,
                                           float raw, float mask_a_val) {
    float c = lfd_cert_floor(raw, L.kp.certainty_thresh);
    if (S.ref.mask_a) c = c * mask_a_val;
    const uint8_t* mb = S.slot[j].mask_b;
    if (mb) {
        const float2 wv = load_f32x2(S.slot[j].warp + (size_t)cell * L.warp_channels + (L.warp_channels - 2));
        const int ix = lfd_grid_nearest(wv.x, L.W);
        const int iy = lfd_grid_nearest(wv.y, L.H);
        float m = 0.0f;
        if (ix >= 0 && iy >= 0)
            m = (float)lfd_global(mb)[(size_t)lfd_nearest_src(iy, L.mask_sy, L.h_match) * L.w_match + lfd_nearest_src(ix, L.mask_sx, L.w_match)];
        c = c * m;
    }
    return c;
}

__device__ __forceinline__ float cell_mask_a(const LfdLaunch& L, const BlockShared& S, int x, int y) {
    if (!S.ref.mask_a) return 1.0f;
    return (float)lfd_global(S.ref.mask_a)[(size_t)lfd_nearest_src(y, L.mask_sy, L.h_match) * L.w_match + lfd_nearest_src(x, L.mask_sx, L.w_match)];
}

__device__ __forceinline__ void argmax_step(float c, int j, float& best, int& bj) {
    const bool take = (c > best) || ((c != c) && !(best != best));
    if (take) { best = c; bj = j; }
}

__device__ __forceinline__ void cell_best(const LfdLaunch& L, const BlockShared& S, int cell, float& best, int& bj) {
    int y, x;
    lfd_divmod(cell, L.W, L.inv_w, y, x);
    const float ma = cell_mask_a(L, S, x, y);
    const int ns = S.ref.n_slots;
    best = cell_cert(L, S, 0, cell, x, y, lfd_global(S.slot[0].cert)[cell], ma);
    bj = 0;
    for (int j = 1; j < ns; ++j) argmax_step(cell_cert(L, S, j, cell, x, y, lfd_global(S.slot[j].cert)[cell], ma), j, best, bj);
}

__device__ __forceinline__ void cells4_best_masked(const LfdLaunch& L, const BlockShared& S, int cell0, int y, int x0,
                                                   float best[4], int bj[4]) {
    const float th = L.kp.certainty_thresh;
    float ma[4] = {1.0f, 1.0f, 1.0f, 1.0f};
    const bool has_a = S.ref.mask_a != nullptr;
    if (has_a) {
        const uint8_t LFD_GLOBAL_AS* row = lfd_global(S.ref.mask_a) + (size_t)lfd_nearest_src(y, L.mask_sy, L.h_match) * L.w_match;
#pragma unroll
        for (int e = 0; e < 4; ++e) ma[e] = (float)row[lfd_nearest_src(x0 + e, L.mask_sx, L.w_match)];
    }
    const int ns = S.ref.n_slots;
    for (int j = 0; j < ns; ++j) {
        const float4 c4 = load_f32x4(S.slot[j].cert + cell0);
        float c[4] = {lfd_cert_floor(c4.x, th), lfd_cert_floor(c4.y, th), lfd_cert_floor(c4.z, th), lfd_cert_floor(c4.w, th)};
        if (has_a) {
#pragma unroll
            for (int e = 0; e < 4; ++e) c[e] = c[e] * ma[e];
        }
        const uint8_t* mb = S.slot[j].mask_b;
        if (mb) {
            float wx[4], wy[4];
            const float* wp = S.slot[j].warp;
            if (L.warp_channels == 4) {
#pragma unroll
                for (int e = 0; e < 4; ++e) { const float4 v = load_f32x4(wp + (size_t)(unsigned)(cell0 + e) * 4); wx[e] = v.z; wy[e] = v.w; }
            } else {
                const float4 a = load_f32x4(wp + (size_t)(unsigned)cell0 * 2), b = load_f32x4(wp + (size_t)(unsigned)cell0 * 2 + 4);
                wx[0] = a.x; wy[0] = a.y; wx[1] = a.z; wy[1] = a.w; wx[2] = b.x; wy[2] = b.y; wx[3] = b.z; wy[3] = b.w;
            }
#pragma unroll
            for (int e = 0; e < 4; ++e) {
                const int ix = lfd_grid_nearest(wx[e], L.W);
                const int iy = lfd_grid_nearest(wy[e], L.H);
                float m = 0.0f;
                if (ix >= 0 && iy >= 0)
                    m = (float)lfd_global(mb)[(size_t)lfd_nearest_src(iy, L.mask_sy, L.h_match) * L.w_match + lfd_nearest_src(ix, L.mask_sx, L.w_match)];
                c[e] = c[e] * m;
            }
        }
        if (j == 0) {
#pragma unroll
            for (int e = 0; e < 4; ++e) { best[e] = c[e]; bj[e] = 0; }
        } else {
#pragma unroll
            for (int e = 0; e < 4; ++e) argmax_step(c[e], j, best[e], bj[e]);
        }
    }
}

__device__ __forceinline__ void cell_coords(const LfdLaunch& L, const BlockShared& S, int cell, int bj, float& xan,
                                            float& yan, float& xbn, float& ybn) {
    const float* wp = S.slot[bj].warp;
    if (L.warp_channels == 4) {
        const float4 v = load_f32x4(wp + (size_t)cell * 4);
        xan = v.x; yan = v.y; xbn = v.z; ybn = v.w;
    } else {
        const float2 v = load_f32x2(wp + (size_t)cell * 2);
        int y, x;
        lfd_divmod(cell, L.W, L.inv_w, y, x);
        xan = lfd_global(L.axis_x)[x]; yan = lfd_global(L.axis_y)[y];
        xbn = v.x; ybn = v.y;
    }
}

}

extern "C" __global__ void lfd_pair_setup_kernel(LfdLaunch L, LfdRefConst* __restrict__ ref_out,
                                                 LfdPairConst* __restrict__ pair_out) {
    const int i = (int)(blockIdx.x * blockDim.x + threadIdx.x);
    const int n_pairs = L.n_refs * L.k;
    if (i < n_pairs) {
        const int r = i / L.k, j = i - r * L.k;
        if (j < L.refs[r].n_slots) {
            lfd_make_pair_const(L.cams[L.refs[r].cam], L.cams[L.slots[i].cam], L.slots[i].cam, L.w_match, L.h_match, pair_out[i],
                                L.fund_override ? L.fund_override + (size_t)i * 9 : nullptr);
        }
    } else if (i < n_pairs + L.n_refs) {
        const int r = i - n_pairs;
        lfd_make_ref_const(L.cams[L.refs[r].cam], L.w_match, L.h_match, ref_out[r]);
    }
}

extern "C" __global__ void __launch_bounds__(256) lfd_aggregate_kernel(LfdLaunch L, float* __restrict__ best_cert,
                                                                       uint8_t* __restrict__ best_slot) {
    __shared__ BlockShared S;
    const int r = (int)blockIdx.y;
    const int tid = (int)threadIdx.x;
    if (tid == 0) S.ref = L.refs[r];
    if (tid < L.k) S.slot[tid] = L.slots[(size_t)r * L.k + tid];
    __syncthreads();
    const int HW = L.H * L.W;
    const bool plain = !S.ref.mask_a && (HW & 3) == 0;
    bool any_mask_b = false;
    for (int j = 0; j < S.ref.n_slots; ++j) any_mask_b |= (S.slot[j].mask_b != nullptr);
    const int ns = S.ref.n_slots;
    for (int base = ((int)blockIdx.x * 256 + tid) * 4; base < HW; base += (int)gridDim.x * 256 * 4) {
        if (plain && !any_mask_b && base + 3 < HW) {
            float4 best = load_f32x4(S.slot[0].cert + base);
            const float th = L.kp.certainty_thresh;
            best.x = lfd_cert_floor(best.x, th); best.y = lfd_cert_floor(best.y, th);
            best.z = lfd_cert_floor(best.z, th); best.w = lfd_cert_floor(best.w, th);
            int b0 = 0, b1 = 0, b2 = 0, b3 = 0;
            for (int j = 1; j < ns; ++j) {
                const float4 c = load_f32x4(S.slot[j].cert + base);
                argmax_step(lfd_cert_floor(c.x, th), j, best.x, b0);
                argmax_step(lfd_cert_floor(c.y, th), j, best.y, b1);
                argmax_step(lfd_cert_floor(c.z, th), j, best.z, b2);
                argmax_step(lfd_cert_floor(c.w, th), j, best.w, b3);
            }
            *reinterpret_cast<float4*>(best_cert + (size_t)r * HW + base) = best;
            if (best_slot) {
                const unsigned packed = (unsigned)b0 | ((unsigned)b1 << 8) | ((unsigned)b2 << 16) | ((unsigned)b3 << 24);
                *reinterpret_cast<unsigned*>(best_slot + (size_t)r * HW + base) = packed;
            }
        } else if ((L.W & 3) == 0 && (HW & 3) == 0 && base + 3 < HW) {
            int y, x0;
            lfd_divmod(base, L.W, L.inv_w, y, x0);
            float b4[4]; int j4[4];
            cells4_best_masked(L, S, base, y, x0, b4, j4);
            *reinterpret_cast<float4*>(best_cert + (size_t)r * HW + base) = make_float4(b4[0], b4[1], b4[2], b4[3]);
            if (best_slot) {
                const unsigned packed = (unsigned)j4[0] | ((unsigned)j4[1] << 8) | ((unsigned)j4[2] << 16) | ((unsigned)j4[3] << 24);
                *reinterpret_cast<unsigned*>(best_slot + (size_t)r * HW + base) = packed;
            }
        } else {
            for (int e = 0; e < 4 && base + e < HW; ++e) {
                float best; int bj;
                cell_best(L, S, base + e, best, bj);
                best_cert[(size_t)r * HW + base + e] = best;
                if (best_slot) best_slot[(size_t)r * HW + base + e] = (uint8_t)bj;
            }
        }
    }
}

#define LFD_CONST_AS __attribute__((address_space(4)))
template <class T>
__device__ __forceinline__ const T LFD_CONST_AS* lfd_const_as(const T* p) {
#pragma clang diagnostic push
#pragma clang diagnostic ignored "-Wold-style-cast"
    return (const T LFD_CONST_AS*)p;
#pragma clang diagnostic pop
}

__device__ __forceinline__ int lfd_slot_bytes12(int sl) {
    int o;
    asm("v_mul_u32_u24 %0, %1, 12" : "=v"(o) : "v"(sl));
    return o;
}

struct DenseStage {
    float xyz[3 * kTile];
    float err[kTile];
    unsigned char slot[kTile];
};

struct __attribute__((packed, aligned(4))) LfdF3 { float a, b, c; };

constexpr int kCopyThreadsOrdered = kBlock - 64;

#if defined(LFD_DENSE_TIMING)
#define LFD_STAMP(i) do { if (L.phase_stamps && lane == 0 && wave < 2) L.phase_stamps[((size_t)blockIdx.x * 2 + wave) * 12 + (i)] = __builtin_readcyclecounter(); } while (0)
#else
#define LFD_STAMP(i) do { } while (0)
#endif

template <bool kExactColour, bool kUnordered = false, bool kPly = false>
__device__ __forceinline__ void lfd_dense_body(const LfdLaunch& L) {
    struct DenseShared {
        BlockShared S;
        DenseStage stage;
        u64 tile_excl;
        unsigned ticket;
        unsigned wave_cnt[kBlock / 64];
        unsigned slot_cnt[LFD_MAX_SLOTS];
    };
    __shared__ DenseShared sh;
    BlockShared& S = sh.S;
    DenseStage& stage = sh.stage;
    static_assert(sizeof(sh.S.pc) >= kTile * sizeof(unsigned short), "the order map does not fit the per-pair constant block");
    unsigned short* const stage_order = reinterpret_cast<unsigned short*>(sh.S.pc);
    unsigned& s_ticket = sh.ticket;
    unsigned (&s_wave_cnt)[kBlock / 64] = sh.wave_cnt;
    unsigned (&s_slot_cnt)[LFD_MAX_SLOTS] = sh.slot_cnt;
    u64& s_tile_excl = sh.tile_excl;

    const int tid = (int)threadIdx.x;
    const int lane = tid & 63, wave = tid >> 6;
#if defined(LFD_DENSE_TIMING)
#endif
    LFD_STAMP(0);
    const unsigned seq = blockIdx.x % LFD_TICKET_LANES;
    const unsigned n_tiles = (unsigned)L.n_refs * (unsigned)L.tiles_per_ref;
    const int HW = L.H * L.W;

#if LFD_STAGGER_UNITS > 0
    if (blockIdx.x < (unsigned)LFD_DENSE_WAVES_PER_SIMD * 256u) {
        const unsigned slot = blockIdx.x >> 8;
        for (unsigned i = 0; i < slot; ++i) __builtin_amdgcn_s_sleep(LFD_STAGGER_UNITS);
    }
#endif
    const unsigned tile_guess = blockIdx.x;
    const int r_guess = __builtin_amdgcn_readfirstlane((int)(tile_guess / (unsigned)L.tiles_per_ref));
#if LFD_FRONT_PRIO > 0
    __builtin_amdgcn_s_setprio(LFD_FRONT_PRIO);
#endif
    PrologueRegs pro;
    if (tile_guess < n_tiles) prologue_issue(L, r_guess, pro);
    if (tid == 0) {
        const unsigned long long k = atomicAdd(L.ticket_lanes + (size_t)seq * 16, 1ull) - L.ticket_base_lane[seq];
        s_ticket = (unsigned)k * LFD_TICKET_LANES + seq;
    }
    if (tid < LFD_MAX_SLOTS) s_slot_cnt[tid] = 0;
    if (tile_guess < n_tiles) prologue_commit(L, pro, S);
    __syncthreads();
    LFD_STAMP(1);
    const unsigned tile = s_ticket;
    if (tile == 0 && (L.seg_counts || kUnordered)) {
        if (L.seg_counts) for (int i = tid; i < L.n_refs * L.k; i += kBlock) L.seg_counts[i] = 0;
        if (kUnordered) for (int i = tid; i < L.n_refs; i += kBlock) L.ref_cursor[i] = 0ull;
        __threadfence();
        __syncthreads();
        if (tid == 0) __hip_atomic_store(L.seg_ready, L.epoch, __ATOMIC_RELEASE, __HIP_MEMORY_SCOPE_AGENT);
    }
    if (tile < n_tiles) {
        const int r = __builtin_amdgcn_readfirstlane((int)(tile / (unsigned)L.tiles_per_ref));
        const int tile_in_ref = (int)(tile - (unsigned)r * (unsigned)L.tiles_per_ref);
        LfdRefConst rc;
        {
            const LfdRefConst LFD_CONST_AS* rcp = lfd_const_as(L.ref_const) + r;
#pragma unroll
            for (int i = 0; i < 12; ++i) rc.P[i] = rcp->P[i];
#pragma unroll
            for (int i = 0; i < 3; ++i) rc.C[i] = rcp->C[i];
            rc.sx = rcp->sx; rc.sy = rcp->sy; rc.pad = 0.0f;
        }
        if (r != r_guess || tile_guess >= n_tiles) {
            __syncthreads();
            block_prologue(L, r, S);
        }
        LFD_STAMP(2);
#if defined(LFD_DENSE_TIMING)
        if (L.phase_stamps && lane == 0 && wave < 2) {
            unsigned long long* s0 = L.phase_stamps + ((size_t)blockIdx.x * 2 + wave) * 12;
            *s0 = (*s0 & ~3ull) | (r == r_guess ? 1ull : 0ull) | (tile == tile_guess ? 2ull : 0ull);
        }
#endif
        const int ns = S.ref.n_slots;
        const bool any_mask = S.ref.any_mask != 0;
        const int tile_cell0 = tile_in_ref * kTile;
        const int cell0 = tile_cell0 + tid * kCpt;
        int tile_y0, tile_x0;
        {
            int ty, tx;
            lfd_divmod(tile_cell0, L.W, L.inv_w, ty, tx);
            tile_y0 = __builtin_amdgcn_readfirstlane(ty); tile_x0 = __builtin_amdgcn_readfirstlane(tx);
        }

        int bj[kCpt];
        unsigned dead = 0;
#if LFD_DENSE_ALL_WARPS
        float spec_xb[4] = {0.0f, 0.0f, 0.0f, 0.0f}, spec_yb[4] = {0.0f, 0.0f, 0.0f, 0.0f};
        bool have_warps = false;
        if (!any_mask && (HW & 3) == 0 && kCpt == 4 && cell0 + 3 < HW && ns <= LFD_DENSE_ALL_WARPS && L.warp_channels == 2) {
            const float th = L.kp.certainty_thresh;
            float4 c[4], wa[4], wb[4];
#pragma unroll
            for (int j = 0; j < 4; ++j) {
                if (j < ns) {
                    c[j] = load_f32x4(S.slot[j].cert + cell0);
                    wa[j] = load_f32x4(S.slot[j].warp + (size_t)(unsigned)cell0 * 2);
                    wb[j] = load_f32x4(S.slot[j].warp + (size_t)(unsigned)cell0 * 2 + 4);
                }
            }
            float4 best = c[0];
            best.x = lfd_cert_floor(best.x, th); best.y = lfd_cert_floor(best.y, th);
            best.z = lfd_cert_floor(best.z, th); best.w = lfd_cert_floor(best.w, th);
            bj[0] = bj[1] = bj[2] = bj[3] = 0;
            spec_xb[0] = wa[0].x; spec_yb[0] = wa[0].y; spec_xb[1] = wa[0].z; spec_yb[1] = wa[0].w;
            spec_xb[2] = wb[0].x; spec_yb[2] = wb[0].y; spec_xb[3] = wb[0].z; spec_yb[3] = wb[0].w;
#pragma unroll
            for (int j = 1; j < 4; ++j) {
                if (j < ns) {
                    int t;
                    t = bj[0]; argmax_step(lfd_cert_floor(c[j].x, th), j, best.x, bj[0]); if (bj[0] != t) { spec_xb[0] = wa[j].x; spec_yb[0] = wa[j].y; }
                    t = bj[1]; argmax_step(lfd_cert_floor(c[j].y, th), j, best.y, bj[1]); if (bj[1] != t) { spec_xb[1] = wa[j].z; spec_yb[1] = wa[j].w; }
// ... 338 lines not shown
                    for (int v = 0; v < LFD_COPY_UNROLL; ++v) {
                        if (u0 + v >= kCopyRecords) break;
#if defined(LFD_ABLATE_COLOUR)
                        rgb[u0 + v][0] = px[v]; rgb[u0 + v][1] = py[v]; rgb[u0 + v][2] = (float)(taps[v].r0 + taps[v].r1 + sh0[v] + sh1[v]);
#else
                        if (kExactColour) lfd_bilinear_eval(taps[v], sh0[v], sh1[v], L.w_match, L.h_match, px[v], py[v], rgb[u0 + v]);
                        else lfd_bilinear_eval_f32(taps[v], sh0[v], sh1[v], L.w_match, L.h_match, px[v], py[v], rgb[u0 + v]);
#endif
                    }
                }
            }
            }
#endif
        }
        if (kUnordered && tid == 0) {
            s_tile_excl = (u64)(unsigned)r * (u64)(unsigned)HW + claimed;
            LfdTileSeg seg; seg.offset = (int32_t)claimed; seg.count = (int32_t)block_total;
            L.tile_table[tile] = seg;
        }
        LFD_STAMP(8);
        __syncthreads();
        LFD_STAMP(9);

#if !defined(LFD_ABLATE_STORES)
        if (kUnordered || wave != 0) {
            const u64 excl = s_tile_excl;
            const long long base = (long long)(((u64)(unsigned)__builtin_amdgcn_readfirstlane((int)(unsigned)(excl >> 32)) << 32) |
                                               (u64)(unsigned)__builtin_amdgcn_readfirstlane((int)(unsigned)excl));
            long long room = L.capacity - base;
            int n = (int)block_total;
            if (room < (long long)n) n = room > 0 ? (int)room : 0;
            if (kPly) {
                unsigned char* gp = L.ply + 15 * base;
#pragma unroll
                for (int u = 0; u < kCopyRecords; ++u) {
                    const int i = ctid + u * kCopyThreads;
                    if (i < n) {
                        const int sl = (int)stage_order[i];
                        const float* sxyz = reinterpret_cast<const float*>(reinterpret_cast<const unsigned char*>(stage.xyz) + lfd_slot_bytes12(sl));
                        struct __attribute__((packed, aligned(1))) F3u { float a, b, c; };
                        struct __attribute__((packed, aligned(1))) U16u { unsigned short v; };
                        F3u p; p.a = sxyz[0]; p.b = sxyz[1]; p.c = sxyz[2];
                        const unsigned o15 = (unsigned)i * 15u;
                        const unsigned q0 = lfd_quantise_u8(rgb[u][0]), q1 = lfd_quantise_u8(rgb[u][1]), q2 = lfd_quantise_u8(rgb[u][2]);
                        *reinterpret_cast<F3u*>(gp + o15) = p;
                        U16u rg; rg.v = (unsigned short)(q0 | (q1 << 8));
                        *reinterpret_cast<U16u*>(gp + o15 + 12u) = rg;
                        gp[o15 + 14u] = (unsigned char)q2;
                        if (L.cell) L.cell[base + i] = tile_cell0 + sl;
                        if (L.slot) L.slot[base + i] = stage.slot[sl];
                    }
                }
            } else {
            unsigned char* gx = reinterpret_cast<unsigned char*>(L.xyz + 3 * base);
            unsigned char* gc = reinterpret_cast<unsigned char*>(L.rgb + 3 * base);
            unsigned char* ge = reinterpret_cast<unsigned char*>(L.err + base);
#pragma unroll
            for (int u = 0; u < kCopyRecords; ++u) {
                const int i = ctid + u * kCopyThreads;
                if (i < n) {
                    const int sl = (int)stage_order[i];
                    LfdF3 p, c;
                    const float* sxyz = reinterpret_cast<const float*>(reinterpret_cast<const unsigned char*>(stage.xyz) + lfd_slot_bytes12(sl));
                    p.a = sxyz[0]; p.b = sxyz[1]; p.c = sxyz[2];
                    c.a = rgb[u][0]; c.b = rgb[u][1]; c.c = rgb[u][2];
                    const unsigned o12 = (unsigned)lfd_slot_bytes12(i), o4 = (unsigned)i * 4u;
#if LFD_NT_STORES
                    float* fx = reinterpret_cast<float*>(gx + o12);
                    float* fc = reinterpret_cast<float*>(gc + o12);
                    __builtin_nontemporal_store(p.a, fx); __builtin_nontemporal_store(p.b, fx + 1); __builtin_nontemporal_store(p.c, fx + 2);
                    __builtin_nontemporal_store(c.a, fc); __builtin_nontemporal_store(c.b, fc + 1); __builtin_nontemporal_store(c.c, fc + 2);
                    __builtin_nontemporal_store(stage.err[sl], reinterpret_cast<float*>(ge + o4));
#else
                    *reinterpret_cast<LfdF3*>(gx + o12) = p;
                    *reinterpret_cast<LfdF3*>(gc + o12) = c;
                    *reinterpret_cast<float*>(ge + o4) = stage.err[sl];
#endif
                    if (L.cell) L.cell[base + i] = tile_cell0 + sl;
                    if (L.slot) L.slot[base + i] = stage.slot[sl];
                }
            }
        }
#endif
            }
#if defined(LFD_DENSE_TIMING)
        LFD_STAMP(10);
        if (L.phase_stamps && lane == 0 && wave < 2) {
            asm volatile("s_waitcnt vmcnt(0)" ::: "memory");
            L.phase_stamps[((size_t)blockIdx.x * 2 + wave) * 12 + 11] = __builtin_readcyclecounter();
        }
#endif
    }
}

extern "C" __global__ void __launch_bounds__(kBlock, LFD_DENSE_WAVES_PER_SIMD) lfd_dense_kernel(LfdLaunch L) { lfd_dense_body<false>(L); }
extern "C" __global__ void __launch_bounds__(kBlock, LFD_DENSE_WAVES_PER_SIMD) lfd_dense_exact_kernel(LfdLaunch L) { lfd_dense_body<true>(L); }
extern "C" __global__ void __launch_bounds__(kBlock, LFD_DENSE_WAVES_PER_SIMD) lfd_dense_ply_kernel(LfdLaunch L) { lfd_dense_body<false, false, true>(L); }
extern "C" __global__ void __launch_bounds__(kBlock, LFD_DENSE_WAVES_PER_SIMD) lfd_dense_ply_exact_kernel(LfdLaunch L) { lfd_dense_body<true, false, true>(L); }
extern "C" __global__ void __launch_bounds__(kBlock, LFD_DENSE_WAVES_PER_SIMD) lfd_dense_segments_kernel(LfdLaunch L) { lfd_dense_body<false, true>(L); }
extern "C" __global__ void __launch_bounds__(kBlock, LFD_DENSE_WAVES_PER_SIMD) lfd_dense_segments_exact_kernel(LfdLaunch L) { lfd_dense_body<true, true>(L); }
extern "C" __global__ void __launch_bounds__(kBlock, LFD_DENSE_WAVES_PER_SIMD) lfd_dense_ply_segments_kernel(LfdLaunch L) { lfd_dense_body<false, true, true>(L); }
extern "C" __global__ void __launch_bounds__(kBlock, LFD_DENSE_WAVES_PER_SIMD) lfd_dense_ply_segments_exact_kernel(LfdLaunch L) { lfd_dense_body<true, true, true>(L); }

extern "C" __global__ void __launch_bounds__(LFD_INDEXED_EVAL_BLOCK) lfd_indexed_eval_kernel(LfdLaunch L, const long long* __restrict__ sel_idx,
                                                                                             const long long* __restrict__ sel_offsets,
                                                                                             float* __restrict__ scratch, uint8_t* __restrict__ codes,
                                                                                             unsigned* __restrict__ tab, int off_pairs) {
    __shared__ BlockShared S;
    __shared__ unsigned s_cnt[LFD_MAX_SLOTS];
    __shared__ unsigned s_first[LFD_MAX_SLOTS];
    const int tid = (int)threadIdx.x;
    const int r = (int)blockIdx.y;
    const long long sel_begin = off_pairs ? sel_offsets[2 * r] : sel_offsets[r], sel_end = off_pairs ? sel_offsets[2 * r + 1] : sel_offsets[r + 1];
    const int n_sel = (int)(sel_end - sel_begin);
    const int i = (int)blockIdx.x * LFD_INDEXED_EVAL_BLOCK + tid;
    if ((int)blockIdx.x * LFD_INDEXED_EVAL_BLOCK >= n_sel) return;
    if (tid < LFD_MAX_SLOTS) { s_cnt[tid] = 0; s_first[tid] = 0xffffffffu; }
    block_prologue(L, r, S);
    const int HW = L.H * L.W;
    if (i < n_sel) {
        const long long cl = sel_idx[sel_begin + i];
        unsigned code = 0xffu;
        if (cl >= 0 && cl < HW) {
            const int cell = (int)cl;
            float best; int bj;
            cell_best(L, S, cell, best, bj);
            float xan, yan, xbn, ybn;
            cell_coords(L, S, cell, bj, xan, yan, xbn, ybn);
            LfdCellResult res;
            lfd_eval_correspondence(S.rc, S.pc[bj], xan, yan, xbn, ybn, L.kp, res);
            atomicMin(&s_first[bj], (unsigned)i);
            code = (unsigned)bj | (res.keep ? 0x80u : 0u);
            if (res.keep) {
                float rgb[3];
                lfd_bilinear_rgb(S.ref.image, L.w_match, L.h_match, res.xa_px, res.ya_px, 1.0f, 1.0f, rgb);
                float* o = scratch + (size_t)(sel_begin + i) * 8;
                o[0] = res.x; o[1] = res.y; o[2] = res.z; o[3] = res.err; o[4] = rgb[0]; o[5] = rgb[1]; o[6] = rgb[2];
                atomicAdd(&s_cnt[bj], 1u);
            }
        }
        codes[sel_begin + i] = (uint8_t)code;
    }
    __syncthreads();
    if (tid < LFD_MAX_SLOTS) {
        unsigned* t = tab + ((size_t)r * LFD_MAX_SLOTS + tid) * 2;
        if (s_cnt[tid]) atomicAdd(t + 0, s_cnt[tid]);
        if (s_first[tid] != 0xffffffffu) atomicMax(t + 1, 0xffffffffu - s_first[tid]);
    }
}

extern "C" __global__ void __launch_bounds__(LFD_INDEXED_BLOCK) lfd_indexed_kernel(LfdLaunch L, const long long* __restrict__ sel_idx,
                                                                                   const long long* __restrict__ sel_offsets,
                                                                                   float* __restrict__ scratch, uint8_t* __restrict__ codes,
                                                                                   int32_t* __restrict__ seg_order, const unsigned* __restrict__ tab, int off_pairs) {
    __shared__ BlockShared S;
    __shared__ unsigned s_ticket;
    __shared__ unsigned s_cnt[LFD_MAX_SLOTS];
    __shared__ unsigned s_first[LFD_MAX_SLOTS];
    __shared__ unsigned s_start[LFD_MAX_SLOTS];
    __shared__ unsigned s_run[LFD_MAX_SLOTS];
    __shared__ unsigned s_wcnt[LFD_INDEXED_BLOCK / 64][LFD_MAX_SLOTS];
    __shared__ u64 s_excl;
    __shared__ unsigned s_total;

    const int tid = (int)threadIdx.x, lane = tid & 63, wave = tid >> 6;
    constexpr int nwaves = LFD_INDEXED_BLOCK / 64;
    if (tid == 0) s_ticket = (unsigned)(atomicAdd(L.ticket, 1ull) - L.ticket_base);
    if (tid < LFD_MAX_SLOTS) { s_cnt[tid] = 0; s_first[tid] = 0xffffffffu; s_run[tid] = 0; }
    __syncthreads();
    const int r = (int)s_ticket;
    block_prologue(L, r, S);
    const int ns = S.ref.n_slots;
    const long long sel_begin = off_pairs ? sel_offsets[2 * r] : sel_offsets[r], sel_end = off_pairs ? sel_offsets[2 * r + 1] : sel_offsets[r + 1];
    const int n_sel = (int)(sel_end - sel_begin);
    const int HW = L.H * L.W;

    if (tab) {
        if (tid < LFD_MAX_SLOTS) {
            s_cnt[tid] = tab[((size_t)r * LFD_MAX_SLOTS + tid) * 2 + 0];
            s_first[tid] = 0xffffffffu - tab[((size_t)r * LFD_MAX_SLOTS + tid) * 2 + 1];
        }
    }
    for (int i = tid; i < (tab ? 0 : n_sel); i += LFD_INDEXED_BLOCK) {
        const long long cl = sel_idx[sel_begin + i];
        unsigned code = 0xffu;
        if (cl >= 0 && cl < HW) {
            const int cell = (int)cl;
            float best; int bj;
            cell_best(L, S, cell, best, bj);
            float xan, yan, xbn, ybn;
            cell_coords(L, S, cell, bj, xan, yan, xbn, ybn);
            LfdCellResult res;
            lfd_eval_correspondence(S.rc, S.pc[bj], xan, yan, xbn, ybn, L.kp, res);
            atomicMin(&s_first[bj], (unsigned)i);
            code = (unsigned)bj | (res.keep ? 0x80u : 0u);
            if (res.keep) {
                float rgb[3];
                lfd_bilinear_rgb(S.ref.image, L.w_match, L.h_match, res.xa_px, res.ya_px, 1.0f, 1.0f, rgb);
                float* o = scratch + (size_t)(sel_begin + i) * 8;
                o[0] = res.x; o[1] = res.y; o[2] = res.z; o[3] = res.err; o[4] = rgb[0]; o[5] = rgb[1]; o[6] = rgb[2];
                atomicAdd(&s_cnt[bj], 1u);
            }
        }
        codes[sel_begin + i] = (uint8_t)code;
    }
    __syncthreads();

    if (tid == 0) {
        unsigned total = 0;
        int g = 0;
        bool used[LFD_MAX_SLOTS];
        for (int j = 0; j < LFD_MAX_SLOTS; ++j) used[j] = false;
        for (int round = 0; round < ns; ++round) {
            int pick = -1; unsigned fp = 0xffffffffu;
            for (int j = 0; j < ns; ++j) if (!used[j] && s_first[j] < fp) { fp = s_first[j]; pick = j; }
            if (pick < 0) break;
            used[pick] = true;
            s_start[pick] = total;
            total += s_cnt[pick];
            if (s_cnt[pick]) { if (seg_order) seg_order[(size_t)r * L.k + g] = pick; ++g; }
        }
        if (seg_order) for (; g < L.k; ++g) seg_order[(size_t)r * L.k + g] = -1;
        s_total = total;
    }
    if (L.seg_counts && tid < L.k) L.seg_counts[(size_t)r * L.k + tid] = (tid < ns) ? (int)s_cnt[tid] : 0;
    __syncthreads();
    if (wave == 0) {
        const u64 excl = lookback_exclusive(L, (unsigned)r, s_total);
        if (lane == 0) {
            s_excl = excl;
            L.ref_offsets[r] = (long long)excl;
            if (r == L.n_refs - 1) L.ref_offsets[L.n_refs] = (long long)(excl + s_total);
        }
    }
    __syncthreads();

    const long long out_base = (long long)s_excl;
    for (int round0 = 0; round0 < n_sel; round0 += LFD_INDEXED_BLOCK) {
        const int i = round0 + tid;
        unsigned code = 0xffu;
        if (i < n_sel) code = codes[sel_begin + i];
        const bool kept = (code != 0xffu) && (code & 0x80u);
        const int j = (int)(code & 0x7fu);
        unsigned rank_in_wave = 0;
        for (int jj = 0; jj < ns; ++jj) {
            const u64 m = __ballot(kept && j == jj);
            if (lane == 0) s_wcnt[wave][jj] = (unsigned)__popcll(m);
            if (kept && j == jj) rank_in_wave = (unsigned)__popcll(m & ((1ull << lane) - 1ull));
        }
        __syncthreads();
        if (kept) {
            unsigned before = s_run[j];
            for (int w = 0; w < wave; ++w) before += s_wcnt[w][j];
            const long long pos = out_base + s_start[j] + before + rank_in_wave;
            if (pos < L.capacity) {
                const float* o = scratch + (size_t)(sel_begin + i) * 8;
                L.xyz[pos * 3 + 0] = o[0]; L.xyz[pos * 3 + 1] = o[1]; L.xyz[pos * 3 + 2] = o[2];
                L.err[pos] = o[3];
                L.rgb[pos * 3 + 0] = o[4]; L.rgb[pos * 3 + 1] = o[5]; L.rgb[pos * 3 + 2] = o[6];
                if (L.cell) L.cell[pos] = (int32_t)sel_idx[sel_begin + i];
                if (L.slot) L.slot[pos] = (uint8_t)j;
            }
        }
        __syncthreads();
        if (tid < ns) {
            unsigned add = 0;
            for (int w = 0; w < nwaves; ++w) add += s_wcnt[w][tid];
            s_run[tid] += add;
        }
        __syncthreads();
    }
}
```

### lichtfeld-densification-plugin_amd/csrc/lfd_select.hip

```cpp
#include <hip/hip_runtime.h>
#include <stdint.h>

#include "lfd_device.hpp"

namespace {

constexpr int kSelBlock = LFD_SELECT_BLOCK;
#ifndef LFD_PRODUCER_PIECE
#define LFD_PRODUCER_PIECE 4096
#endif
constexpr int kScanRoundDraws = 1024;

__device__ __forceinline__ unsigned mt_temper(unsigned y) {
    y ^= (y >> 11);
    y ^= (y << 7) & 0x9d2c5680u;
    y ^= (y << 15) & 0xefc60000u;
    y ^= (y >> 18);
    return y;
}

__device__ void mt_twist_lds(const unsigned* o, unsigned* n, int tid) {
    auto mix = [](unsigned a, unsigned b) { const unsigned y = (a & 0x80000000u) | (b & 0x7fffffffu); return (y >> 1) ^ ((y & 1u) ? 0x9908b0dfu : 0u); };
    if (tid < 227) n[tid] = o[tid + 397] ^ mix(o[tid], o[tid + 1]);
    __syncthreads();
// ... 1209 lines not shown
    }
    LFD_MW_STAMP();
#undef LFD_MW_STAMP
#undef LFD_GRID_SYNC
#undef LFD_CHAIN_PASS
#undef LFD_CHAIN_BREAK
}

namespace {

__device__ __forceinline__ unsigned topm_ord(float c, float cap) {
    c = (c > cap) ? cap : c;
    const unsigned u = __float_as_uint(c);
    if (c != c) return 0u;
    unsigned ord = (u & 0x80000000u) ? ~u : (u | 0x80000000u);
    if (ord == 0u) ord = 1u;
    return ord;
}

__device__ int topm_pick_bin(const unsigned* hist, int n_bins, unsigned need, int* s_i, int* s_pick, int tid, unsigned& need_out) {
    const int b_hi = n_bins - 1 - 2 * tid, b_lo = b_hi - 1;
    const unsigned h_hi = b_hi >= 0 ? hist[b_hi] : 0u, h_lo = b_lo >= 0 ? hist[b_lo] : 0u;
    int total;
    const int excl = block_excl_scan_i32((int)(h_hi + h_lo), s_i, tid, total);
    if ((unsigned)excl < need && need <= (unsigned)excl + h_hi + h_lo) {
        if (need <= (unsigned)excl + h_hi) { s_pick[0] = b_hi; s_pick[1] = (int)(need - (unsigned)excl); }
        else { s_pick[0] = b_lo; s_pick[1] = (int)(need - (unsigned)excl - h_hi); }
    }
    __syncthreads();
    need_out = (unsigned)s_pick[1];
    return s_pick[0];
}

}

extern "C" __global__ void __launch_bounds__(LFD_SELECT_BLOCK) lfd_select_topm_kernel(LfdSelectArgs A_launch) {
    const LfdSelectArgs A = lfd_select_args_of(A_launch);
    extern __shared__ __attribute__((aligned(16))) unsigned long long s_keys[];
    __shared__ unsigned s_hist[2048];
    __shared__ unsigned s_count;
    __shared__ int s_i[kSelBlock / 64];
    __shared__ int s_pick[2];
    __shared__ int s_wave_ties[kSelBlock / 64];

    const int tid = (int)threadIdx.x, lane = tid & 63, wave = tid >> 6;
    const int N = A.H * A.W;
    const int M = min(A.M, N);
    if (tid == 0) { *A.n_out = 0; *A.status = LFD_SELECT_OK; }
    if (M <= 0) return;
    if (M > LFD_SELECT_TOPM_MAX || (long long)M > A.capacity) { if (tid == 0) *A.status = LFD_SELECT_CAPACITY; return; }
    const float* cert = A.best_cert;
    const float cap = A.cap;
    const bool vec4 = ((N & 3) == 0) && ((reinterpret_cast<uintptr_t>(cert) & 15u) == 0);

    auto for_each_cell = [&](auto&& f) {
        if (vec4) {
#pragma unroll 4
            for (int g = tid; g < (N >> 2); g += kSelBlock) {
                const float4 c4 = *reinterpret_cast<const float4*>(cert + 4 * g);
                f(4 * g + 0, topm_ord(c4.x, cap)); f(4 * g + 1, topm_ord(c4.y, cap));
                f(4 * g + 2, topm_ord(c4.z, cap)); f(4 * g + 3, topm_ord(c4.w, cap));
            }
        } else {
#pragma unroll 4
            for (int i = tid; i < N; i += kSelBlock) f(i, topm_ord(cert[i], cap));
        }
    };

    unsigned need = (unsigned)M;
    for (int b = tid; b < 2048; b += kSelBlock) s_hist[b] = 0;
    __syncthreads();
    for_each_cell([&](int, unsigned ord) { atomicAdd(&s_hist[ord >> 21], 1u); });
    __syncthreads();
    const unsigned d2 = (unsigned)topm_pick_bin(s_hist, 2048, need, s_i, s_pick, tid, need);
    __syncthreads();
    for (int b = tid; b < 2048; b += kSelBlock) s_hist[b] = 0;
    __syncthreads();
    for_each_cell([&](int, unsigned ord) { if ((ord >> 21) == d2) atomicAdd(&s_hist[(ord >> 10) & 0x7ffu], 1u); });
    __syncthreads();
    const unsigned d1 = (unsigned)topm_pick_bin(s_hist, 2048, need, s_i, s_pick, tid, need);
    __syncthreads();
    for (int b = tid; b < 2048; b += kSelBlock) s_hist[b] = 0;
    __syncthreads();
    const unsigned hi21 = (d2 << 11) | d1;
    for_each_cell([&](int, unsigned ord) { if ((ord >> 10) == hi21) atomicAdd(&s_hist[ord & 0x3ffu], 1u); });
    __syncthreads();
    const unsigned d0 = (unsigned)topm_pick_bin(s_hist, 1024, need, s_i, s_pick, tid, need);
    const unsigned ord_k = (hi21 << 10) | d0;
    const unsigned ties = s_hist[d0];
    __syncthreads();

    if (tid == 0) s_count = 0;
    __syncthreads();
    if (need >= ties) {
        for_each_cell([&](int i, unsigned ord) {
            if (ord >= ord_k) { const unsigned pos = atomicAdd(&s_count, 1u); if (pos < (unsigned)LFD_SELECT_TOPM_MAX) s_keys[pos] = ((unsigned long long)ord << 32) | (unsigned long long)(0xffffffffu - (unsigned)i); }
        });
    } else {
        constexpr int nwaves = kSelBlock / 64;
        const int span = ((N + nwaves - 1) / nwaves + 255) & ~255;
        const int w_lo = min(wave * span, N), w_hi = min(w_lo + span, N);
        int my_ties = 0;
#pragma unroll 4
        for (int i = w_lo + 4 * lane; i < w_hi; i += 256)
            for (int e = 0; e < 4 && i + e < w_hi; ++e) my_ties += topm_ord(cert[i + e], cap) == ord_k;
#pragma unroll
        for (int off = 32; off > 0; off >>= 1) my_ties += __shfl_xor(my_ties, off, 64);
        if (lane == 0) s_wave_ties[wave] = my_ties;
        __syncthreads();
        unsigned rank_base = 0;
        for (int w = 0; w < wave; ++w) rank_base += (unsigned)s_wave_ties[w];
        for (int base = w_lo; base < w_hi; base += 256) {
            const int i0 = base + 4 * lane;
            unsigned ords[4];
            int t = 0;
#pragma unroll
            for (int e = 0; e < 4; ++e) { ords[e] = (i0 + e < w_hi) ? topm_ord(cert[i0 + e], cap) : 0u; t += (i0 + e < w_hi) && ords[e] == ord_k; }
            int incl = t;
#pragma unroll
            for (int off = 1; off < 64; off <<= 1) { const int n = __shfl_up(incl, off, 64); if (lane >= off) incl += n; }
            unsigned r = rank_base + (unsigned)(incl - t);
#pragma unroll
            for (int e = 0; e < 4; ++e) {
                if (i0 + e >= w_hi) continue;
                bool take = ords[e] > ord_k;
                if (ords[e] == ord_k) { take = r < need; ++r; }
                if (take) { const unsigned pos = atomicAdd(&s_count, 1u); if (pos < (unsigned)LFD_SELECT_TOPM_MAX) s_keys[pos] = ((unsigned long long)ords[e] << 32) | (unsigned long long)(0xffffffffu - (unsigned)(i0 + e)); }
            }
            rank_base += (unsigned)__shfl(incl, 63, 64);
        }
    }
    __syncthreads();
    int P = 1;
    while (P < M) P <<= 1;
    for (int i = M + tid; i < P; i += kSelBlock) s_keys[i] = 0ull;
    __syncthreads();
    for (int k = 2; k <= P; k <<= 1) {
        for (int j = k >> 1; j > 0; j >>= 1) {
            for (int i = tid; i < P; i += kSelBlock) {
                const int l = i ^ j;
                if (l > i) {
                    const unsigned long long a = s_keys[i], b = s_keys[l];
                    const bool desc = ((i & k) == 0);
                    if (desc ? (a < b) : (a > b)) { s_keys[i] = b; s_keys[l] = a; }
                }
            }
            __syncthreads();
        }
    }
    for (int i = tid; i < M; i += kSelBlock) A.sel_out[i] = (long long)(0xffffffffu - (unsigned)(s_keys[i] & 0xffffffffull));
    if (tid == 0) { *A.n_out = M; if (A.sel_offsets_out) A.sel_offsets_out[1] = A.sel_offsets_out[0] + M; }
}

extern "C" __global__ void lfd_select_begins_kernel(long long* pairs, long long stride, int n) {
    const int r = (int)(blockIdx.x * blockDim.x + threadIdx.x);
    if (r < n) { pairs[2 * r] = (long long)r * stride; pairs[2 * r + 1] = (long long)r * stride; }
}

extern "C" __global__ void lfd_mt_seed_kernel(unsigned* mt, unsigned seed) {
    if (threadIdx.x == 0 && blockIdx.x == 0) {
        mt[0] = seed;
        for (int i = 1; i < 624; ++i) mt[i] = 1812433253u * (mt[i - 1] ^ (mt[i - 1] >> 30)) + (unsigned)i;
        mt[624] = 624;
    }
}

extern "C" __global__ void lfd_mt_seed_batch_kernel(unsigned* mt_base, LfdSeedBatch seeds) {
    if (threadIdx.x == 0) {
        unsigned* mt = mt_base + (size_t)blockIdx.x * LFD_MT_STATE_STRIDE;
        mt[0] = seeds.seed[blockIdx.x];
        for (int i = 1; i < 624; ++i) mt[i] = 1812433253u * (mt[i - 1] ^ (mt[i - 1] >> 30)) + (unsigned)i;
        mt[624] = 624;
    }
}
```

Measured before the change: 51.72 billion.

## Fold pair setup, scratch clearing and begin offsets into the aggregate kernel

The certainty aggregate kernel now also takes over several small launches in the sampled path. When needed it runs the per-pair constant setup in extra blocks, and its first block writes the selection begin offsets and zeroes the index table and the cooperative/chain scratch. This removes the separate pair-setup kernel, the begins kernel and the memsets before selection. The cost is more work in the aggregate kernel, a reworked scratch reservation via a SelectPlan helper, and a status readback hook in the indexed kernel. A profiling script is also added.

```diff
diff --git a/lichtfeld-densification-plugin_amd/csrc/lfd_api.hip b/lichtfeld-densification-plugin_amd/csrc/lfd_api.hip
--- a/lichtfeld-densification-plugin_amd/csrc/lfd_api.hip
+++ b/lichtfeld-densification-plugin_amd/csrc/lfd_api.hip
@@ -28,6 +28,8 @@
 #include "lfd_cap.hpp"
 
 extern "C" __global__ void lfd_aggregate_kernel(LfdLaunch L, float* best_cert, uint8_t* best_slot);
+extern "C" __global__ void lfd_aggregate_fold_kernel(LfdLaunch L, float* best_cert, uint8_t* best_slot, LfdAggFold F);
+extern "C" __global__ void lfd_aggregate_setup_kernel(LfdLaunch L, float* best_cert, uint8_t* best_slot, LfdAggFold F);
 extern "C" __global__ void lfd_dense_kernel(LfdLaunch L);
 extern "C" __global__ void lfd_dense_exact_kernel(LfdLaunch L);
 extern "C" __global__ void lfd_dense_ply_kernel(LfdLaunch L);
@@ -126,13 +128,12 @@
 extern "C" __global__ void lfd_pack_ply_normals_kernel(const float* xyz, const float* normals, const float* rgb, long long n, unsigned char* out);
 extern "C" __global__ void lfd_select_topm_kernel(LfdSelectArgs A);
 extern "C" __global__ void lfd_select_filter_mw_kernel(LfdSelectArgs A, LfdSelectNorms norms);
-extern "C" __global__ void lfd_select_begins_kernel(long long* pairs, long long stride, int n);
 extern "C" __global__ void lfd_mt_seed_kernel(unsigned* mt, unsigned seed);
 extern "C" __global__ void lfd_mt_seed_batch_kernel(unsigned* mt_base, LfdSeedBatch seeds);
 extern "C" __global__ void lfd_indexed_eval_kernel(LfdLaunch L, const long long* sel_idx, const long long* sel_offsets, float* scratch,
                                                    uint8_t* codes, unsigned* tab, int off_pairs);
 extern "C" __global__ void lfd_indexed_kernel(LfdLaunch L, const long long* sel_idx, const long long* sel_offsets,
-                                              float* scratch, uint8_t* codes, int32_t* seg_order, const unsigned* tab, int off_pairs);
+                                              float* scratch, uint8_t* codes, int32_t* seg_order, const unsigned* tab, int off_pairs, int* status_out);
 
 namespace {
 
@@ -367,8 +368,20 @@
 
 namespace {
 
+int consts_derived(lfd_context* ctx, LfdBatchSlot& sl, const lfd_batch* b, hipStream_t st) {
+    sl.consts_valid = true;
+    sl.refs = b->n_refs; sl.k = b->k;
+    sl.wm = b->w_match;
+    sl.hm = b->h_match;
+    if (st != ctx->stream) {
+        LFD_HIP(ctx, hipEventRecord(sl.ready, st));
+        sl.ready_pending = true;
+    }
+    return LFD_OK;
+}
+
 int prepare_launch(lfd_context* ctx, const lfd_batch* b, const lfd_params* p, const long long* extra, size_t n_extra,
-                   LfdLaunch& L, const long long** d_extra, bool ahead = false) {
+                   LfdLaunch& L, const long long** d_extra, bool ahead = false, bool* fold_setup = nullptr) {
     int rc = validate_batch(ctx, b, p);
     if (rc != LFD_OK) return rc;
     LFD_HIP(ctx, hipSetDevice(ctx->device));
@@ -414,17 +427,17 @@
     LfdPairConst* d_pc = reinterpret_cast<LfdPairConst*>(static_cast<unsigned char*>(sl.consts.ptr) + ref_bytes);
     L.ref_const = d_rc;
     L.pair_const = d_pc;
+    if (fold_setup) *fold_setup = false;
     if (!sl.consts_valid || sl.wm != b->w_match || sl.hm != b->h_match) {
-        const int n = b->n_refs * b->k + b->n_refs;
-        hipLaunchKernelGGL(lfd_pair_setup_kernel, dim3((unsigned)((n + 63) / 64)), dim3(64), 0, st, L, d_rc, d_pc);
-        LFD_HIP(ctx, hipGetLastError());
-        sl.consts_valid = true;
-        sl.refs = b->n_refs; sl.k = b->k;
-        sl.wm = b->w_match;
-        sl.hm = b->h_match;
-        if (st != ctx->stream) {
-            LFD_HIP(ctx, hipEventRecord(sl.ready, st));
-            sl.ready_pending = true;
+        if (fold_setup && st == ctx->stream) {
+            sl.consts_valid = false;
+            *fold_setup = true;
+        } else {
+            const int n = b->n_refs * b->k + b->n_refs;
+            hipLaunchKernelGGL(lfd_pair_setup_kernel, dim3((unsigned)((n + 63) / 64)), dim3(64), 0, st, L, d_rc, d_pc);
+            LFD_HIP(ctx, hipGetLastError());
+            rc = consts_derived(ctx, sl, b, st);
+            if (rc != LFD_OK) return rc;
         }
     }
     if (!ahead) {
@@ -1070,7 +1083,7 @@
     }
     hipLaunchKernelGGL(lfd_indexed_kernel, dim3((unsigned)batch->n_refs), dim3(LFD_INDEXED_BLOCK), 0, ctx->stream, L,
                        reinterpret_cast<const long long*>(sel_idx), d_off, static_cast<float*>(ctx->scratch.ptr),
-                       static_cast<uint8_t*>(ctx->codes.ptr), seg_order, static_cast<const unsigned*>(tab), 0);
+                       static_cast<uint8_t*>(ctx->codes.ptr), seg_order, static_cast<const unsigned*>(tab), 0, static_cast<int*>(nullptr));
     LFD_HIP(ctx, hipGetLastError());
     return LFD_OK;
 }
@@ -1141,10 +1154,53 @@
     return n_wg >= 2 && ctx->env.select_timing == 0;
 }
 
+struct SelectPlan {
+    size_t o_w, o_p, o_cdf, o_first, o_mark, o_draws, o_cand, o_found, o_out, o_time, o_coop, total;
+    bool timing, several_wg;
+    int n_wg;
+    long long ring_cap;
+    int snap_slots, n_chains;
+    size_t o_ring, o_snaps, chain_total;
+};
+
+static SelectPlan select_plan(lfd_context* ctx, bool topm, int32_t H, int32_t W, int32_t M, int n_batch, bool one_stream) {
+    SelectPlan P;
+    std::memset(&P, 0, sizeof(P));
+    const size_t N = (size_t)H * W, Mz = (size_t)std::max(M, 1);
+    auto up = [](size_t v) { return (v + 255) & ~size_t(255); };
+    P.o_w = 0; P.o_p = P.o_w + up(N * 4); P.o_cdf = P.o_p + up(N * 8); P.o_first = P.o_cdf + up(N * 8); P.o_mark = P.o_first + up(N * 4);
+    P.o_draws = P.o_mark + up(N); P.o_cand = P.o_draws + up(Mz * 8); P.o_found = P.o_cand + up(Mz * 4); P.o_out = P.o_found + up(Mz * 4);
+    P.o_time = P.o_out + 256; P.o_coop = P.o_time + 256; P.total = P.o_coop + up(LFD_SELECT_COOP_BYTES);
+    P.timing = !topm && n_batch == 1 && ctx->env.select_timing != 0;
+    if (topm) return P;
+    int n_wg = LFD_SELECT_DEFAULT_WG;
+    if (ctx->env.select_workgroups >= 0) n_wg = ctx->env.select_workgroups;
+    P.n_wg = std::min(std::min(n_wg, (int)LFD_SELECT_MAX_WG), (int)(N / 8192));
+    const bool timing_mw = P.timing && ctx->env.select_timing == 2;
+    P.several_wg = P.n_wg >= 2 && (!P.timing || timing_mw);
+    if (P.several_wg) {
+        const long long first_round = std::max<long long>(std::min<long long>((long long)((double)M * 0.85), (long long)N), 1);
+        P.ring_cap = 4096;
+        while (P.ring_cap < 4 * first_round) P.ring_cap *= 2;
+        P.snap_slots = (int)(2 * P.ring_cap / 624) + 8;
+        P.o_ring = LFD_CHAIN_BYTES; P.o_snaps = P.o_ring + (size_t)P.ring_cap * 8;
+        P.chain_total = (P.o_snaps + (size_t)P.snap_slots * 624 * 4 + 255) & ~size_t(255);
+        P.n_chains = one_stream ? 1 : n_batch;
+    }
+    return P;
+}
+
+static int select_reserve(lfd_context* ctx, const SelectPlan& P, int n_batch) {
+    int rc = ensure(ctx, ctx->sel_scratch, P.total * (size_t)n_batch);
+    if (rc != LFD_OK) return rc;
+    if (P.several_wg) rc = ensure(ctx, ctx->sel_chain, P.chain_total * (size_t)P.n_chains);
+    return rc;
+}
+
 static int select_launch(lfd_context* ctx, bool topm, const float* best_cert, int32_t H, int32_t W, int32_t M, float cap,
                          int32_t border, int32_t tiles, float s_override, int64_t* sel_out, int64_t capacity,
                          long long* sel_offsets_dev, int** d_info, unsigned char** d_time, int n_batch = 1,
-                         unsigned* mt_batch = nullptr, int* info_batch = nullptr, const float* s_batch = nullptr) {
+                         unsigned* mt_batch = nullptr, int* info_batch = nullptr, const float* s_batch = nullptr, bool cleared = false) {
     if (!ctx) return fail(nullptr, LFD_ERR_INVALID, "null context");
     if (!best_cert || !sel_out) return fail(ctx, LFD_ERR_INVALID, "null argument");
     if (ctx->is_host) return fail(ctx, LFD_ERR_STATE, "device entry point called on a host context");
@@ -1154,11 +1210,11 @@
     if (n_batch < 1 || n_batch > LFD_SELECT_BATCH_MAX) return fail(ctx, LFD_ERR_INVALID, "bad selection batch");
     LFD_HIP(ctx, hipSetDevice(ctx->device));
     if (!ctx->mt.ptr) { int rc0 = ensure(ctx, ctx->mt, 625 * sizeof(unsigned)); if (rc0 != LFD_OK) return rc0; }
-    const size_t N = (size_t)H * W, Mz = (size_t)std::max(M, 1);
-    auto up = [](size_t v) { return (v + 255) & ~size_t(255); };
-    const size_t o_w = 0, o_p = o_w + up(N * 4), o_cdf = o_p + up(N * 8), o_first = o_cdf + up(N * 8), o_mark = o_first + up(N * 4),
-                 o_draws = o_mark + up(N), o_cand = o_draws + up(Mz * 8), o_found = o_cand + up(Mz * 4), o_out = o_found + up(Mz * 4),
-                 o_time = o_out + 256, o_coop = o_time + 256, total = o_coop + up(LFD_SELECT_COOP_BYTES);
+    const size_t N = (size_t)H * W;
+    const bool one_stream = mt_batch == nullptr;
+    const SelectPlan P = select_plan(ctx, topm, H, W, M, n_batch, one_stream);
+    const size_t o_w = P.o_w, o_p = P.o_p, o_cdf = P.o_cdf, o_first = P.o_first, o_mark = P.o_mark, o_draws = P.o_draws, o_cand = P.o_cand,
+                 o_found = P.o_found, o_out = P.o_out, o_time = P.o_time, o_coop = P.o_coop, total = P.total;
     int rc = ensure(ctx, ctx->sel_scratch, total * (size_t)n_batch);
     if (rc != LFD_OK) return rc;
     unsigned char* base = static_cast<unsigned char*>(ctx->sel_scratch.ptr);
@@ -1193,7 +1249,7 @@
     }
     *d_info = reinterpret_cast<int*>(base + o_out);
     *d_time = nullptr;
-    const bool timing = !topm && n_batch == 1 && ctx->env.select_timing != 0;
+    const bool timing = P.timing;
     if (timing) {
         A.timing = reinterpret_cast<unsigned long long*>(base + o_time);
         LFD_HIP(ctx, hipMemsetAsync(base + o_time, 0, 256, ctx->stream));
@@ -1208,9 +1264,7 @@
         }
         hipLaunchKernelGGL(lfd_select_topm_kernel, dim3(1, (unsigned)n_batch), dim3(LFD_SELECT_BLOCK), lds, ctx->stream, A);
     } else {
-        int n_wg = LFD_SELECT_DEFAULT_WG;
-        if (ctx->env.select_workgroups >= 0) n_wg = ctx->env.select_workgroups;
-        n_wg = std::min(std::min(n_wg, (int)LFD_SELECT_MAX_WG), (int)(N / 8192));
+        const int n_wg = P.n_wg;
         {
             const int tile = std::max(1, W / tiles);
             const long long nbins = (long long)((W - 1) / tile + 1) * ((H - 1) / tile + 1);
@@ -1220,24 +1274,20 @@
                             std::to_string((int)LFD_SELECT_MAX_BINS) + " (every square grid fits; RoMa's, 320 ... 1280 cells per side, have 576 ... 625); the host selection "
                             "stage (selection_backend=\"host\" in the Python mirror: upstream's own library calls) has no such limit");
         }
-        const bool timing_mw = timing && ctx->env.select_timing == 2;
-        const bool several_wg = n_wg >= 2 && (!timing || timing_mw);
-        const bool one_stream = mt_batch == nullptr;
+        const bool several_wg = P.several_wg;
         if (one_stream && n_batch > 1 && !several_wg)
             return fail(ctx, LFD_ERR_STATE, "selection: several references on one stream need the multi-workgroup kernel");
         if (several_wg) {
-            const long long first_round = std::max<long long>(std::min<long long>((long long)((double)M * 0.85), (long long)N), 1);
-            long long ring_cap = 4096;
-            while (ring_cap < 4 * first_round) ring_cap *= 2;
-            const int snap_slots = (int)(2 * ring_cap / 624) + 8;
-            const size_t o_ring = LFD_CHAIN_BYTES, o_snaps = o_ring + (size_t)ring_cap * 8,
-                         chain_total = (o_snaps + (size_t)snap_slots * 624 * 4 + 255) & ~size_t(255);
-            const int n_chains = one_stream ? 1 : n_batch;
+            const long long ring_cap = P.ring_cap;
+            const int snap_slots = P.snap_slots, n_chains = P.n_chains;
+            const size_t o_ring = P.o_ring, o_snaps = P.o_snaps, chain_total = P.chain_total;
             rc = ensure(ctx, ctx->sel_chain, chain_total * (size_t)n_chains);
             if (rc != LFD_OK) return rc;
             unsigned char* cb = static_cast<unsigned char*>(ctx->sel_chain.ptr);
-            if (n_chains == 1) LFD_HIP(ctx, hipMemsetAsync(cb, 0, LFD_CHAIN_BYTES, ctx->stream));
-            else LFD_HIP(ctx, hipMemset2DAsync(cb, chain_total, 0, LFD_CHAIN_BYTES, (size_t)n_chains, ctx->stream));
+            if (!cleared) {
+                if (n_chains == 1) LFD_HIP(ctx, hipMemsetAsync(cb, 0, LFD_CHAIN_BYTES, ctx->stream));
+                else LFD_HIP(ctx, hipMemset2DAsync(cb, chain_total, 0, LFD_CHAIN_BYTES, (size_t)n_chains, ctx->stream));
+            }
             A.chain = cb;
             A.ring = reinterpret_cast<double*>(cb + o_ring);
             A.snaps = reinterpret_cast<unsigned*>(cb + o_snaps);
@@ -1249,8 +1299,10 @@
         if (several_wg) {
             A.coop = base + o_coop;
             A.n_wg = n_wg;
-            if (n_batch == 1) LFD_HIP(ctx, hipMemsetAsync(base + o_coop, 0, LFD_COOP_MT, ctx->stream));
-            else LFD_HIP(ctx, hipMemset2DAsync(base + o_coop, total, 0, LFD_COOP_MT, (size_t)n_batch, ctx->stream));
+            if (!cleared) {
+                if (n_batch == 1) LFD_HIP(ctx, hipMemsetAsync(base + o_coop, 0, LFD_COOP_MT, ctx->stream));
+                else LFD_HIP(ctx, hipMemset2DAsync(base + o_coop, total, 0, LFD_COOP_MT, (size_t)n_batch, ctx->stream));
+            }
             hipLaunchKernelGGL(lfd_select_filter_mw_kernel, dim3((unsigned)n_wg + 1u, (unsigned)n_batch), dim3(LFD_SELECT_BLOCK), 0, ctx->stream, A, norms);
         } else {
             hipLaunchKernelGGL(lfd_select_filter_kernel, dim3(1, (unsigned)n_batch), dim3(LFD_SELECT_BLOCK), 0, ctx->stream, A);
@@ -1307,33 +1359,66 @@
     const bool topm = params->no_filter != 0;
     if (topm && M > LFD_SELECT_TOPM_MAX) return fail(ctx, LFD_ERR_INVALID, "no_filter selection is limited to 16384 matches per reference");
     LfdLaunch L;
-    int rc = prepare_launch(ctx, batch, params, nullptr, 0, L, nullptr);
+    bool fold_setup = false;
+    int rc = prepare_launch(ctx, batch, params, nullptr, 0, L, nullptr, false, &fold_setup);
     if (rc != LFD_OK) return rc;
     rc = check_points(ctx, out, reinterpret_cast<long long*>(ref_offsets));
     if (rc != LFD_OK) return rc;
     const long long HW = (long long)batch->H * batch->W;
     const long long cap_sel = topm ? std::max<long long>(std::min<long long>(M, HW), 1) : (long long)M + (long long)tiles * tiles + 64;
     if (out->capacity < cap_sel * R) return fail(ctx, LFD_ERR_CAPACITY, "output capacity below (M + tiles*tiles + 64) per reference");
+    rc = ensure(ctx, ctx->sel_buf, (size_t)R * 16 + (size_t)cap_sel * (size_t)R * sizeof(long long));
+    if (rc != LFD_OK) return rc;
+    long long* sel_pairs = static_cast<long long*>(ctx->sel_buf.ptr);
+    long long* cells = sel_cells ? reinterpret_cast<long long*>(sel_cells) : sel_pairs + 2 * (size_t)R;
+    const size_t tab_bytes = (size_t)R * LFD_MAX_SLOTS * 2 * sizeof(unsigned);
+    rc = ensure(ctx, ctx->idx_tab, tab_bytes);
+    if (rc != LFD_OK) return rc;
+    unsigned* tab = static_cast<unsigned*>(ctx->idx_tab.ptr);
+    const bool batched = !seeds && (topm || select_runs_on_several_workgroups(ctx, HW)) && R > 1;
+    const int nb0 = (batched || seeds) ? std::min(R, (int)LFD_SELECT_BATCH_MAX) : 1;
     rc = ensure(ctx, ctx->agg, (size_t)HW * (size_t)R * sizeof(float));
     if (rc != LFD_OK) return rc;
     float* best = static_cast<float*>(ctx->agg.ptr);
     {
+        const SelectPlan P0 = select_plan(ctx, topm, batch->H, batch->W, M, nb0, !seeds);
+        rc = select_reserve(ctx, P0, nb0);
+        if (rc != LFD_OK) return rc;
+        LfdAggFold F;
+        std::memset(&F, 0, sizeof(F));
+        F.pairs = sel_pairs;
+        F.pair_stride = R == 1 ? 0 : cap_sel;
+        F.tab = tab;
+        if (P0.several_wg) {
+            F.coop = static_cast<unsigned char*>(ctx->sel_scratch.ptr) + P0.o_coop;
+            F.coop_stride = (long long)P0.total;
+            F.coop_refs = nb0;
+            F.chain = static_cast<unsigned char*>(ctx->sel_chain.ptr);
+            F.chain_stride = (long long)P0.chain_total;
+            F.chain_refs = P0.n_chains;
+        }
         const int per_block = 256 * 4;
         const int gx = (int)std::min<long long>((HW + per_block - 1) / per_block, 2048);
-        hipLaunchKernelGGL(lfd_aggregate_kernel, dim3((unsigned)gx, (unsigned)R, 1u), dim3(256), 0, ctx->stream, L, best, static_cast<uint8_t*>(nullptr));
+        int gx_setup = 0;
+        if (fold_setup) {
+            gx_setup = (R * batch->k + R + 255) / 256;
+            F.agg_blocks = gx;
+            F.ref_out = const_cast<LfdRefConst*>(L.ref_const);
+            F.pair_out = const_cast<LfdPairConst*>(L.pair_const);
+        }
+        if (fold_setup)
+            hipLaunchKernelGGL(lfd_aggregate_setup_kernel, dim3((unsigned)(gx + gx_setup), (unsigned)R, 1u), dim3(256), 0, ctx->stream, L, best,
+                               static_cast<uint8_t*>(nullptr), F);
+        else
+            hipLaunchKernelGGL(lfd_aggregate_fold_kernel, dim3((unsigned)gx, (unsigned)R, 1u), dim3(256), 0, ctx->stream, L, best,
+                               static_cast<uint8_t*>(nullptr), F);
         LFD_HIP(ctx, hipGetLastError());
-    }
-    rc = ensure(ctx, ctx->sel_buf, (size_t)R * 16 + (size_t)cap_sel * (size_t)R * sizeof(long long));
-    if (rc != LFD_OK) return rc;
-    long long* sel_pairs = static_cast<long long*>(ctx->sel_buf.ptr);
-    long long* cells = sel_cells ? reinterpret_cast<long long*>(sel_cells) : sel_pairs + 2 * (size_t)R;
-    if (R == 1) {
-        LFD_HIP(ctx, hipMemsetAsync(sel_pairs, 0, 16, ctx->stream));
-    } else {
-        hipLaunchKernelGGL(lfd_select_begins_kernel, dim3((unsigned)((R + 255) / 256)), dim3(256), 0, ctx->stream, sel_pairs, (long long)cap_sel, R);
-        LFD_HIP(ctx, hipGetLastError());
-    }
-    if (!seeds && (topm || select_runs_on_several_workgroups(ctx, HW)) && R > 1) {
+        if (fold_setup) {
+            rc = consts_derived(ctx, ctx->slot[ctx->cur], batch, ctx->stream);
+            if (rc != LFD_OK) return rc;
+        }
+    }
+    if (batched) {
         if (!topm && !ctx->mt_seeded) return fail(ctx, LFD_ERR_STATE, "lfd_rng_seed must be called before lfd_triangulate_sampled_chain");
         for (int r0 = 0; r0 < R; r0 += LFD_SELECT_BATCH_MAX) {
             const int nb = std::min(R - r0, (int)LFD_SELECT_BATCH_MAX);
@@ -1341,7 +1426,7 @@
             unsigned char* d_time = nullptr;
             rc = select_launch(ctx, topm, best + (size_t)r0 * HW, batch->H, batch->W, M, cap, topm ? 0 : border, topm ? 1 : tiles, 0.0f,
                                reinterpret_cast<int64_t*>(cells + (size_t)r0 * cap_sel), cap_sel, sel_pairs + 2 * (size_t)r0, &d_info, &d_time,
-                               nb, nullptr, sel_info + 2 * (size_t)r0, (s_chain && !topm) ? s_chain + r0 : nullptr);
+                               nb, nullptr, sel_info + 2 * (size_t)r0, (s_chain && !topm) ? s_chain + r0 : nullptr, r0 == 0);
             if (rc != LFD_OK) return rc;
         }
     } else if (!seeds) {
@@ -1350,9 +1435,9 @@
             unsigned char* d_time = nullptr;
             const float s_r = topm ? 0.0f : (s_chain ? s_chain[r] : s_override);
             rc = select_launch(ctx, topm, best + (size_t)r * HW, batch->H, batch->W, M, cap, topm ? 0 : border, topm ? 1 : tiles, s_r,
-                               reinterpret_cast<int64_t*>(cells + (size_t)r * cap_sel), cap_sel, sel_pairs + 2 * (size_t)r, &d_info, &d_time);
+                               reinterpret_cast<int64_t*>(cells + (size_t)r * cap_sel), cap_sel, sel_pairs + 2 * (size_t)r, &d_info, &d_time,
+                               1, nullptr, sel_info + 2 * (size_t)r, nullptr, r == 0);
             if (rc != LFD_OK) return rc;
-            LFD_HIP(ctx, hipMemcpyAsync(sel_info + 2 * (size_t)r, d_info, 2 * sizeof(int), hipMemcpyDeviceToDevice, ctx->stream));
         }
     } else {
         rc = ensure(ctx, ctx->mt_batch, (size_t)LFD_SELECT_BATCH_MAX * LFD_MT_STATE_STRIDE * sizeof(unsigned));
@@ -1371,7 +1456,7 @@
             unsigned char* d_time = nullptr;
             rc = select_launch(ctx, topm, best + (size_t)r0 * HW, batch->H, batch->W, M, cap, topm ? 0 : border, topm ? 1 : tiles, 0.0f,
                                reinterpret_cast<int64_t*>(cells + (size_t)r0 * cap_sel), cap_sel, sel_pairs + 2 * (size_t)r0, &d_info, &d_time,
-                               nb, mtb, sel_info + 2 * (size_t)r0);
+                               nb, mtb, sel_info + 2 * (size_t)r0, nullptr, r0 == 0);
             if (rc != LFD_OK) return rc;
         }
     }
@@ -1381,11 +1466,6 @@
     if (rc != LFD_OK) return rc;
     rc = ensure(ctx, ctx->codes, (size_t)cap_sel * (size_t)R);
     if (rc != LFD_OK) return rc;
-    const size_t tab_bytes = (size_t)R * LFD_MAX_SLOTS * 2 * sizeof(unsigned);
-    rc = ensure(ctx, ctx->idx_tab, tab_bytes);
-    if (rc != LFD_OK) return rc;
-    unsigned* tab = static_cast<unsigned*>(ctx->idx_tab.ptr);
-    LFD_HIP(ctx, hipMemsetAsync(tab, 0, tab_bytes, ctx->stream));
     L.xyz = out->xyz; L.rgb = out->rgb; L.err = out->err; L.cell = out->cell; L.slot = out->slot;
     L.capacity = out->capacity;
     L.ref_offsets = reinterpret_cast<long long*>(ref_offsets);
@@ -1397,9 +1477,10 @@
     LFD_HIP(ctx, hipGetLastError());
     hipLaunchKernelGGL(lfd_indexed_kernel, dim3((unsigned)R), dim3(LFD_INDEXED_BLOCK), 0, ctx->stream, L,
                        static_cast<const long long*>(cells), static_cast<const long long*>(sel_pairs), static_cast<float*>(ctx->scratch.ptr),
-                       static_cast<uint8_t*>(ctx->codes.ptr), seg_order, static_cast<const unsigned*>(tab), 1);
+                       static_cast<uint8_t*>(ctx->codes.ptr), seg_order, static_cast<const unsigned*>(tab), 1, R == 1 ? sel_info + 2 : nullptr);
     LFD_HIP(ctx, hipGetLastError());
-    LFD_HIP(ctx, hipMemcpyAsync(sel_info + 2 * (size_t)R, static_cast<unsigned char*>(ctx->ws.ptr) + 8, sizeof(int), hipMemcpyDeviceToDevice, ctx->stream));
+    if (R > 1)
+        LFD_HIP(ctx, hipMemcpyAsync(sel_info + 2 * (size_t)R, static_cast<unsigned char*>(ctx->ws.ptr) + 8, sizeof(int), hipMemcpyDeviceToDevice, ctx->stream));
     return LFD_OK;
 }
 
diff --git a/lichtfeld-densification-plugin_amd/csrc/lfd_device.hpp b/lichtfeld-densification-plugin_amd/csrc/lfd_device.hpp
--- a/lichtfeld-densification-plugin_amd/csrc/lfd_device.hpp
+++ b/lichtfeld-densification-plugin_amd/csrc/lfd_device.hpp
@@ -218,6 +218,22 @@
 #define LFD_CHAIN_BYTES 1024
 struct LfdSeedBatch { unsigned seed[LFD_SELECT_BATCH_MAX]; };
 
+struct LfdAggFold {
+    long long* pairs;
+    long long pair_stride;
+    unsigned* tab;
+    unsigned char* coop;
+    long long coop_stride;
+    int coop_refs;
+    int chain_refs;
+    unsigned char* chain;
+    long long chain_stride;
+    int agg_blocks;
+    int pad;
+    LfdRefConst* ref_out;
+    LfdPairConst* pair_out;
+};
+
 #if defined(__HIPCC__)
 #include "lfd_support.hpp"
 
diff --git a/lichtfeld-densification-plugin_amd/csrc/lfd_kernels.hip b/lichtfeld-densification-plugin_amd/csrc/lfd_kernels.hip
--- a/lichtfeld-densification-plugin_amd/csrc/lfd_kernels.hip
+++ b/lichtfeld-densification-plugin_amd/csrc/lfd_kernels.hip
@@ -319,9 +319,7 @@
 
 }
 
-extern "C" __global__ void lfd_pair_setup_kernel(LfdLaunch L, LfdRefConst* __restrict__ ref_out,
-                                                 LfdPairConst* __restrict__ pair_out) {
-    const int i = (int)(blockIdx.x * blockDim.x + threadIdx.x);
+__device__ __forceinline__ void lfd_pair_setup_one(const LfdLaunch& L, int i, LfdRefConst* __restrict__ ref_out, LfdPairConst* __restrict__ pair_out) {
     const int n_pairs = L.n_refs * L.k;
     if (i < n_pairs) {
         const int r = i / L.k, j = i - r * L.k;
@@ -335,11 +333,26 @@
     }
 }
 
-extern "C" __global__ void __launch_bounds__(256) lfd_aggregate_kernel(LfdLaunch L, float* __restrict__ best_cert,
-                                                                       uint8_t* __restrict__ best_slot) {
+extern "C" __global__ void lfd_pair_setup_kernel(LfdLaunch L, LfdRefConst* __restrict__ ref_out,
+                                                 LfdPairConst* __restrict__ pair_out) {
+    lfd_pair_setup_one(L, (int)(blockIdx.x * blockDim.x + threadIdx.x), ref_out, pair_out);
+}
+
+__device__ __forceinline__ void lfd_zero_words(unsigned char* p, long long bytes, int tid) {
+    unsigned long long* q = reinterpret_cast<unsigned long long*>(p);
+    for (long long i = tid; i < bytes / 8; i += 256) q[i] = 0ull;
+}
+
+template <int kFold>
+__device__ __forceinline__ void lfd_aggregate_body(const LfdLaunch& L, float* __restrict__ best_cert, uint8_t* __restrict__ best_slot, const LfdAggFold& F) {
     __shared__ BlockShared S;
     const int r = (int)blockIdx.y;
     const int tid = (int)threadIdx.x;
+    const int agg_blocks = kFold == 2 ? F.agg_blocks : (int)gridDim.x;
+    if (kFold == 2 && (int)blockIdx.x >= agg_blocks) {
+        if (r == 0) lfd_pair_setup_one(L, ((int)blockIdx.x - agg_blocks) * 256 + tid, F.ref_out, F.pair_out);
+        return;
+    }
     if (tid == 0) S.ref = L.refs[r];
     if (tid < L.k) S.slot[tid] = L.slots[(size_t)r * L.k + tid];
     __syncthreads();
@@ -348,7 +361,7 @@
     bool any_mask_b = false;
     for (int j = 0; j < S.ref.n_slots; ++j) any_mask_b |= (S.slot[j].mask_b != nullptr);
     const int ns = S.ref.n_slots;
-    for (int base = ((int)blockIdx.x * 256 + tid) * 4; base < HW; base += (int)gridDim.x * 256 * 4) {
+    for (int base = ((int)blockIdx.x * 256 + tid) * 4; base < HW; base += agg_blocks * 256 * 4) {
         if (plain && !any_mask_b && base + 3 < HW) {
             float4 best = load_f32x4(S.slot[0].cert + base);
             const float th = L.kp.certainty_thresh;
@@ -386,6 +399,25 @@
             }
         }
     }
+    if (kFold != 0 && blockIdx.x == 0) {
+        if (F.pairs && tid == 0) { F.pairs[2 * r] = (long long)r * F.pair_stride; F.pairs[2 * r + 1] = (long long)r * F.pair_stride; }
+        if (F.tab) lfd_zero_words(reinterpret_cast<unsigned char*>(F.tab + (size_t)r * LFD_MAX_SLOTS * 2), LFD_MAX_SLOTS * 2 * sizeof(unsigned), tid);
+        if (r < F.coop_refs) lfd_zero_words(F.coop + (long long)r * F.coop_stride, LFD_COOP_MT, tid);
+        if (r < F.chain_refs) lfd_zero_words(F.chain + (long long)r * F.chain_stride, LFD_CHAIN_BYTES, tid);
+    }
+}
+
+extern "C" __global__ void __launch_bounds__(256) lfd_aggregate_kernel(LfdLaunch L, float* __restrict__ best_cert,
+                                                                       uint8_t* __restrict__ best_slot) {
+    lfd_aggregate_body<0>(L, best_cert, best_slot, LfdAggFold());
+}
+extern "C" __global__ void __launch_bounds__(256) lfd_aggregate_fold_kernel(LfdLaunch L, float* __restrict__ best_cert,
+                                                                            uint8_t* __restrict__ best_slot, LfdAggFold F) {
+    lfd_aggregate_body<1>(L, best_cert, best_slot, F);
+}
+extern "C" __global__ void __launch_bounds__(256) lfd_aggregate_setup_kernel(LfdLaunch L, float* __restrict__ best_cert,
+                                                                             uint8_t* __restrict__ best_slot, LfdAggFold F) {
+    lfd_aggregate_body<2>(L, best_cert, best_slot, F);
 }
 
 #define LFD_CONST_AS __attribute__((address_space(4)))
@@ -1030,7 +1062,8 @@
 extern "C" __global__ void __launch_bounds__(LFD_INDEXED_BLOCK) lfd_indexed_kernel(LfdLaunch L, const long long* __restrict__ sel_idx,
                                                                                    const long long* __restrict__ sel_offsets,
                                                                                    float* __restrict__ scratch, uint8_t* __restrict__ codes,
-                                                                                   int32_t* __restrict__ seg_order, const unsigned* __restrict__ tab, int off_pairs) {
+                                                                                   int32_t* __restrict__ seg_order, const unsigned* __restrict__ tab, int off_pairs,
+                                                                                   int* __restrict__ status_out) {
     __shared__ BlockShared S;
     __shared__ unsigned s_ticket;
     __shared__ unsigned s_cnt[LFD_MAX_SLOTS];
@@ -1109,6 +1142,7 @@
             s_excl = excl;
             L.ref_offsets[r] = (long long)excl;
             if (r == L.n_refs - 1) L.ref_offsets[L.n_refs] = (long long)(excl + s_total);
+            if (status_out) *status_out = (int)__hip_atomic_load(L.status, __ATOMIC_RELAXED, __HIP_MEMORY_SCOPE_AGENT);
         }
     }
     __syncthreads();
diff --git a/lichtfeld-densification-plugin_amd/csrc/lfd_select.hip b/lichtfeld-densification-plugin_amd/csrc/lfd_select.hip
--- a/lichtfeld-densification-plugin_amd/csrc/lfd_select.hip
+++ b/lichtfeld-densification-plugin_amd/csrc/lfd_select.hip
@@ -1385,11 +1385,6 @@
     if (tid == 0) { *A.n_out = M; if (A.sel_offsets_out) A.sel_offsets_out[1] = A.sel_offsets_out[0] + M; }
 }
 
-extern "C" __global__ void lfd_select_begins_kernel(long long* pairs, long long stride, int n) {
-    const int r = (int)(blockIdx.x * blockDim.x + threadIdx.x);
-    if (r < n) { pairs[2 * r] = (long long)r * stride; pairs[2 * r + 1] = (long long)r * stride; }
-}
-
 extern "C" __global__ void lfd_mt_seed_kernel(unsigned* mt, unsigned seed) {
     if (threadIdx.x == 0 && blockIdx.x == 0) {
         mt[0] = seed;
diff --git a/profiles/sampled_commands_time.py b/profiles/sampled_commands_time.py
--- /dev/null
+++ b/profiles/sampled_commands_time.py
@@ -0,0 +1,89 @@
+import argparse
+import json
+import os
+import sys
+
+import torch
+
+sys.path.insert(0, os.path.join(os.path.dirname(os.path.abspath(__file__)), ".."))
+import lichtfeld_densification_plugin_amd as lfd
+from lichtfeld_densification_plugin_amd import synthetic
+from lichtfeld_densification_plugin_amd.core import hip_backend as hb
+
+
+def timed(dev, fn):
+    a, b = torch.cuda.Event(enable_timing=True), torch.cuda.Event(enable_timing=True)
+    torch.cuda.synchronize(dev)
+    a.record()
+    n = fn()
+    b.record()
+    b.synchronize()
+    return a.elapsed_time(b), n
+
+
+def main():
+    ap = argparse.ArgumentParser()
+    ap.add_argument("--passes", type=int, default=5)
+    ap.add_argument("--refs", type=int, default=64)
+    ap.add_argument("--group", type=int, default=16)
+    args = ap.parse_args()
+    H = W = 512
+    k, M, n_cams = 3, 10000, 185
+    dev = torch.device("cuda:0")
+    dens = hb.HipDensifier(dev)
+    cams = synthetic.ring_cameras(n_cams, seed=0)
+    dens.upload_cameras(cams)
+    refs = []
+    for gi in range(args.refs):
+        ref = (gi * 3) % n_cams
+        nbrs = synthetic.ring_neighbours(n_cams, ref, k)
+        s = synthetic.synth_reference(cams, ref, nbrs, H, W, W, H, noise_px=0.5, outlier_frac=0.05, channels=2, seed=1000 + gi, cert_mode="smooth",
+                                      device=dev)
+        refs.append(hb.ReferenceInputs(ref_cam=ref, nbr_cams=nbrs, cert=[s.cert[j] for j in range(k)], warp=[s.warp[j] for j in range(k)], image=s.image))
+    params = hb.make_params(lfd.DensePipelineConfig(output_path="", matches_per_ref=M, nns_per_ref=k))
+    cap = M + 24 * 24 + 64
+    singles = [hb.PreparedBatch([r], W, H) for r in refs]
+    groups = [hb.PreparedBatch(refs[g:g + args.group], W, H) for g in range(0, args.refs, args.group)]
+    out1 = [hb.OutputBuffers(cap, 1, k, dev) for _ in range(2)]
+    outg = [hb.OutputBuffers(cap * args.group, args.group, k, dev) for _ in range(2)]
+
+    def one_per_call():
+        dens.seed_rng(0)
+        n = 0
+        dens.launch_sampled(singles[0], params, M, out1[0])
+        for i in range(len(singles)):
+            if i + 1 < len(singles):
+                dens.launch_sampled(singles[i + 1], params, M, out1[(i + 1) & 1])
+            n += out1[i & 1].collect(indexed=True, check_selection=True).count
+        return n
+
+    def grouped():
+        dens.seed_rng(0)
+        n = 0
+        dens.launch_sampled_chain(groups[0], params, M, outg[0])
+        for i in range(len(groups)):
+            if i + 1 < len(groups):
+                dens.launch_sampled_chain(groups[i + 1], params, M, outg[(i + 1) & 1])
+            n += outg[i & 1].collect(indexed=True, check_selection=True).count
+        return n
+
+    res = {"library": os.environ.get("LFD_DENSIFY_LIB", "(the package's own)"), "refs": args.refs, "group": args.group}
+    for name, fn in (("one_reference_per_call", one_per_call), ("grouped", grouped)):
+        fn()
+        ms, pts = [], None
+        for _ in range(args.passes):
+            dt, n = timed(dev, fn)
+            assert pts is None or n == pts, (n, pts)
+            pts = n
+            ms.append(dt / args.refs)
+        srt = sorted(ms)
+        res[name] = {"ms_per_reference": [round(v, 5) for v in ms], "median": round(srt[len(srt) // 2], 5), "spread": round(srt[-1] - srt[0], 5),
+                     "points": pts}
+        print(f"{name}: median {res[name]['median']:.4f} ms per reference, spread {res[name]['spread']:.4f} over {args.passes} passes "
+              f"({', '.join(f'{v:.4f}' for v in ms)}); {pts} points")
+    print(json.dumps(res))
+    dens.close()
+
+
+if __name__ == "__main__":
+    main()
```

Result: no change. 52.00 billion, median of 3 (+0.5%).
